# MaurizioFD/RecSys2019_DeepLearning_Evaluation

Hardware: NVIDIA B200
Metric: ItemKNN cosine top-K rows/sec (higher is better)
Workload: dtype i32 counts + f32

## Files before the change

### include/b200rec.h

```cpp
#ifndef B200REC_H_
#define B200REC_H_

#include <stdint.h>

#ifdef __cplusplus
extern "C" {
#endif

#define B200_OK 0
#define B200_E_INVALID (-1)
#define B200_E_CUDA (-2)
#define B200_E_NOMEM (-3)
#define B200_E_UNSUPPORTED (-4)

const char* b200_last_error(void);
int b200_version(void);
int64_t b200_launch_count(void);
int b200_device_info(char* name, int name_len, int* sm_count, int64_t* total_mem);

typedef struct b200_sim_s* b200_sim_t;

enum b200_sim_kind {
  B200_SIM_COSINE = 0,
  B200_SIM_ADJUSTED = 1,
  B200_SIM_ASYMMETRIC = 2,
  B200_SIM_PEARSON = 3,
  B200_SIM_JACCARD = 4,
  B200_SIM_DICE = 5,
  B200_SIM_TVERSKY = 6,
  B200_SIM_EUCLIDEAN = 7
};

int b200_sim_create(b200_sim_t* out, int64_t n_rows, int64_t n_cols, int64_t nnz, const int32_t* h_indptr,
                    const int32_t* h_indices, const float* h_data, int kind, int topK, float shrink,
                    int normalize, float asymmetric_alpha, float tversky_alpha, float tversky_beta,
                    const float* h_row_weights, void* stream);
int b200_sim_destroy(b200_sim_t h);

int b200_sim_create_scaled(b200_sim_t* out, int64_t n_rows, int64_t n_cols, int64_t nnz, const int32_t* h_indptr,
                           const int32_t* h_indices, const float* h_data, const float* h_A, const float* h_B,
                           int topK, void* stream);

enum b200_euclid_mode { B200_EUCLID_EXP = 0, B200_EUCLID_LIN = 1, B200_EUCLID_LOG = 2 };
int b200_sim_create_euclidean(b200_sim_t* out, int64_t n_rows, int64_t n_cols, int64_t nnz, const int32_t* h_indptr,
                              const int32_t* h_indices, const float* h_data, int topK, float shrink, int normalize,
                              int normalize_avg_row, int distance_mode, void* stream);

int b200_sim_info(b200_sim_t h, int* K, int* n_windows, int* window_cells, int* binary_path, int* signed_data);

int b200_sim_compute_device(b200_sim_t h, int start_col, int end_col, int32_t* d_idx, float* d_val,
                            int32_t* d_cnt, void* stream);
int b200_sim_compute(b200_sim_t h, int start_col, int end_col, int32_t* h_idx, float* h_val, int32_t* h_cnt);
int b200_sim_compute_peers_device(b200_sim_t h, int start_col, int end_col, int n_tables, void* const* d_tables,
                                  int64_t idx_offset, int64_t val_offset, int64_t cnt_offset, void* stream);
int b200_sim_compute_dense_device(b200_sim_t h, int start_col, int end_col, float* d_out, void* stream);

int b200_topk_table_to_csr_count(int n_cols, int K, const int32_t* d_cnt, int64_t* nnz_out, void* stream);
int b200_topk_table_to_csr_fill(int n_cols, int K, const int32_t* d_idx, const float* d_val,
                                const int32_t* d_cnt, int64_t nnz, int32_t* h_indptr, int32_t* h_indices,
                                float* h_data, void* stream);

int b200_sim_debug_set_cap(b200_sim_t h, int cap);

int b200_sim_debug_phase_cycles(b200_sim_t h, int enable, uint64_t* out8);

int b200_sim_debug_k1c(b200_sim_t h, int set_fail_every, int* enabled, int* ctas_per_sm, int* n_bitmap_cols, int* n_window_cols);

int b200_sim_last_kernel_ms(b200_sim_t h, float* ms);
int b200_sim_work(b200_sim_t h, int start_col, int end_col, int64_t* gathered_entries);
int b200_sim_col_work(b200_sim_t h, int64_t* out_n_cols);

typedef struct b200_mf_s* b200_mf_t;

enum b200_mf_algorithm { B200_MF_BPR = 0, B200_MF_FUNK_SVD = 1 };
enum b200_sgd_mode { B200_SGD = 0, B200_ADAGRAD = 1, B200_RMSPROP = 2, B200_ADAM = 3 };
enum b200_sampler { B200_SAMPLER_GLIBC = 0,
                    B200_SAMPLER_PHILOX = 1  };

int b200_mf_create(b200_mf_t* out, int64_t n_users, int64_t n_items, int64_t nnz, const int32_t* h_indptr,
                   const int32_t* h_indices, const float* h_data, int n_factors, int algorithm, int batch_size,
                   float negative_interactions_quota, float learning_rate, int use_bias, float user_reg,
                   float item_reg, float bias_reg, float positive_reg, float negative_reg, int sgd_mode,
                   float gamma, float beta_1, float beta_2, const double* h_user_factors,
                   const double* h_item_factors, int has_seed, uint32_t random_seed, int sampler, int hogwild);
int b200_mf_destroy(b200_mf_t h);
int b200_mf_epoch(b200_mf_t h, void* stream);
int b200_mf_set_user_shard(b200_mf_t h, int user_lo, int user_hi, int64_t samples_per_epoch, uint32_t stream_id);
int b200_mf_samples_last_epoch(b200_mf_t h, int64_t* n);
int b200_mf_get_samples(b200_mf_t h, int32_t* u, int32_t* i, int32_t* j, float* r);
int b200_mf_get_factors(b200_mf_t h, double* user_factors, double* item_factors, double* user_bias,
                        double* item_bias, double* global_bias);
int b200_mf_device_factors(b200_mf_t h, float** d_user_factors, float** d_item_factors);
int b200_mf_last_epoch_ms(b200_mf_t h, float* ms);
int b200_mf_delta_snapshot_device(const float* d_V, float* d_B, float* d_own, float* d_sum, int64_t n, void* stream);
int b200_mf_delta_apply_device(float* d_V, float* d_B, const float* d_sum, const float* d_own, int64_t n, void* stream);

typedef struct b200_asysvd_s* b200_asysvd_t;
int b200_asysvd_create(b200_asysvd_t* out, int64_t n_users, int64_t n_items, int64_t nnz, const int32_t* h_indptr,
                       const int32_t* h_indices, const float* h_data, int n_factors, double negative_interactions_quota,
                       float learning_rate, int use_bias, float user_reg, float item_reg, float bias_reg, int sgd_mode,
                       float gamma, float beta_1, float beta_2, const double* h_profile_factors,
                       const double* h_item_factors, int has_seed, uint32_t random_seed);
int b200_asysvd_destroy(b200_asysvd_t h);
int b200_asysvd_epoch(b200_asysvd_t h, void* stream);
int b200_asysvd_get_samples(b200_asysvd_t h, int32_t* u, int32_t* i, float* r);
int b200_asysvd_get_factors(b200_asysvd_t h, double* profile_factors, double* item_factors, double* user_bias,
                            double* item_bias, double* global_bias);
int b200_asysvd_last_epoch_ms(b200_asysvd_t h, float* ms);

typedef struct b200_slim_s* b200_slim_t;

int b200_slim_create(b200_slim_t* out, int64_t n_users, int64_t n_items, int64_t nnz, const int32_t* h_indptr,
                     const int32_t* h_indices, float learning_rate, float li_reg, float lj_reg, int symmetric,
                     int sgd_mode, float gamma, float beta_1, float beta_2, int has_seed, uint32_t random_seed,
                     int sampler, int hogwild);
int b200_slim_destroy(b200_slim_t h);
int b200_slim_epoch(b200_slim_t h, void* stream);
int b200_slim_get_samples(b200_slim_t h, int32_t* u, int32_t* i, int32_t* j);
int b200_slim_get_S_dense(b200_slim_t h, float* h_out, float* d_out);
int b200_slim_last_epoch_ms(b200_slim_t h, float* ms);
int b200_slim_enable_tree(b200_slim_t h, int topK);
int b200_slim_tree_prune(b200_slim_t h, int touch_diagonal, void* stream);
int b200_slim_create_sharded(b200_slim_t* out, int64_t n_users, int64_t n_items, int64_t nnz, const int32_t* h_indptr,
                             const int32_t* h_indices, float learning_rate, float li_reg, float lj_reg, int sgd_mode,
                             float gamma, float beta_1, float beta_2, uint32_t random_seed, int col_lo, int col_hi);
int b200_slim_shard_partial_device(b200_slim_t h, int64_t first, int n_batch, float* d_x, void* stream);
int b200_slim_shard_apply_device(b200_slim_t h, int64_t first, int n_batch, const float* d_x_sum, void* stream);
int b200_slim_shard_device(b200_slim_t h, float** d_S, int* col_lo, int* col_hi);

enum b200_topk_mode { B200_TOPK_NONZERO = 0, B200_TOPK_ZEROS_OUTRANK = 1,
                      B200_TOPK_NONZERO_DROP_LAST = 2 };
int b200_dense_topk_device(const float* d_matrix, int n, int K, int along_columns, int mode, int32_t* d_idx,
                           float* d_val, int32_t* d_cnt, void* stream);
int b200_dense_topk_rect_device(const float* d_matrix, int n_lines, int n_inner, int64_t stride_line, int64_t stride_inner,
                                int index_offset, int K, int mode, int32_t* d_idx, float* d_val, int32_t* d_cnt, void* stream);
int b200_sparse_topk_device(int n, const int32_t* d_ptr, const int32_t* d_line_idx, const float* d_vals, int K,
                            int mode, int32_t* d_idx, float* d_val, int32_t* d_cnt, void* stream);

int b200_score_spmm_device(const int32_t* d_users, int n_users_block, const int32_t* d_a_ptr, const int32_t* d_a_idx,
                           const float* d_a_val, const int32_t* d_b_ptr, const int32_t* d_b_idx, const float* d_b_val,
                           int n_out_cols, float* d_out, void* stream);
int b200_transpose_device(const float* d_in, int rows, int cols, float* d_out, void* stream);
int b200_score_mf_device(const int32_t* d_users, int n_users_block, const float* d_user_factors,
                         const float* d_item_factors_T, int n_factors, int n_items, const float* d_user_bias,
                         const float* d_item_bias, const float* d_global_bias, float* d_out, void* stream);
int b200_score_mask_device(const int32_t* d_users, int n_users_block, const int32_t* d_urm_ptr, const int32_t* d_urm_idx,
                           const unsigned char* d_items_keep, int n_items, float* d_scores, void* stream);
int b200_score_topn_device(const float* d_scores, int n_rows, int n_items, int cutoff, int32_t* d_items,
                           float* d_item_scores, void* stream);

int b200_slim_enet_device(const float* d_G, const float* d_diag, int n_items, int64_t n_users, double l1_ratio, double alpha,
                          int positive_only, int max_iter, float tol, float* d_coef_T, int32_t* d_n_iter, void* stream);

int b200_spd_inverse_device(float* d_A, int n_pad, float* d_work, void* stream);
int b200_debug_gemm_device(int version, int kind, int M, int N, int K, float alpha, const float* d_A, int lda,
                           const float* d_B, int ldb, float beta, float* d_C, int ldc, void* stream);
int b200_ease_from_gram_device(const float* d_G, int n_items, const int32_t* d_urm_indices, int64_t nnz, float l2_norm,
                               float* h_B, float* d_B, void* stream);

int b200_ials_half_epoch_device(const int32_t* d_rows, int n_solve, const int32_t* d_ptr, const int32_t* d_idx,
                                const float* d_conf, const double* d_Y, int n_other, int n_factors, double reg,
                                double* d_X, double* d_YtY_work, void* stream);

enum b200_weighting { B200_WEIGHT_BM25 = 0, B200_WEIGHT_TFIDF = 1 };
int b200_feature_weighting_device(int mode, int n_users, int n_items, int64_t nnz, const int32_t* d_indptr,
                                  const int32_t* d_indices, float* d_data, float K1, float B, void* stream);

enum b200_eval_slot {
  B200_EVAL_PRECISION = 0, B200_EVAL_PRECISION_RECALL_MIN_DEN = 1, B200_EVAL_RECALL = 2, B200_EVAL_MAP = 3,
  B200_EVAL_MAP_MIN_DEN = 4, B200_EVAL_MRR = 5, B200_EVAL_NDCG = 6, B200_EVAL_HIT_RATE = 7, B200_EVAL_ARHR = 8,
  B200_EVAL_NOVELTY = 9, B200_EVAL_AVERAGE_POPULARITY = 10, B200_EVAL_USERS_WITH_RECS = 11, B200_EVAL_N_USERS = 12,
  B200_EVAL_NACC = 16
};
int b200_eval_accumulate_device(const int32_t* d_users, int n_block, const int32_t* d_rec_items, const float* d_rec_scores,
                                int max_cutoff, const int32_t* d_test_ptr, const int32_t* d_test_idx,
                                const float* d_test_val, const int32_t* d_cutoffs, int n_cutoffs, const double* d_idcg,
                                const double* d_item_novelty, const double* d_item_pop_norm, int n_items, double* d_acc,
                                int32_t* d_rec_count, int32_t* d_hit_count, void* stream);

#ifdef __cplusplus
}
#endif
#endif
```

### recsys2019_deeplearning_evaluation_b200/csrc/sim_k1d.cuh

```cuda

constexpr int D_THREADS = 512;
constexpr int D_WARPS = D_THREADS / 32;
constexpr int D_ROWS = 4;
constexpr int D_TILE_LOG2 = 10;

struct K1DShared {
  int item, nbuf, cnt, adds, nibsum, tstop, chunk_end, chunk_cnt;
  int need, digit, bincnt, ncand, expect;
  u64 kor, kand;
  int hist[256];
};

__device__ __forceinline__ unsigned nib_ge3(unsigned w) { return (((w | (w >> 1)) >> 2) | (w & (w >> 1))) & 0x11111111u; }
__device__ __forceinline__ unsigned nib_eq2(unsigned w) { return (w >> 1) & ~w & ~(w >> 2) & ~(w >> 3) & 0x11111111u; }
__device__ __forceinline__ unsigned nib_eq1(unsigned w) { return w & ~(w >> 1) & ~(w >> 2) & ~(w >> 3) & 0x11111111u; }
__device__ __forceinline__ unsigned nib_level(unsigned w, int level) {
  return level >= 3 ? nib_ge3(w) : (level == 2 ? nib_eq2(w) : nib_eq1(w));
}
__device__ __forceinline__ int nib_sum(unsigned w) {
  const unsigned b = (w & 0x0F0F0F0Fu) + ((w >> 4) & 0x0F0F0F0Fu);
  return (int)__dp4a(b, 0x01010101u, 0u);
}

__device__ u64 d_select(u64* buf, int n, int K, K1DShared* ds, int* n_out) {
  const int tid = threadIdx.x;
  __syncthreads();
  if (n <= K) { *n_out = n; return 0ull; }
  {
    if (tid == 0) { ds->kor = 0ull; ds->kand = ~0ull; }
    __syncthreads();
    u64 o = 0ull, a = ~0ull;
    for (int q = tid; q < n; q += D_THREADS) { const u64 k = buf[q]; o |= k; a &= k; }
#pragma unroll
    for (int off = 16; off > 0; off >>= 1) { o |= __shfl_xor_sync(0xffffffffu, o, off); a &= __shfl_xor_sync(0xffffffffu, a, off); }
    if ((tid & 31) == 0) { atomicOr(&ds->kor, o); atomicAnd(&ds->kand, a); }
    __syncthreads();
  }
  const u64 diff = ds->kor ^ ds->kand;
  int pass = diff ? (63 - __clzll((long long)diff)) >> 3 : 0;
  u64 prefix = pass < 7 ? (ds->kor >> ((pass + 1) * 8)) << ((pass + 1) * 8) : 0ull;
  int need = K;
  const int one = n > 0 ? 1 : 0;
  for (; pass >= 0; --pass) {
    const int shift = pass * 8;
    if (tid < 256) ds->hist[tid] = 0;
    __syncthreads();
    for (int q = tid; q < n; q += D_THREADS) {
      const u64 k = buf[q];
      if (pass == 7 || (k >> (shift + 8)) == (prefix >> (shift + 8))) atomicAdd(&ds->hist[(int)((k >> shift) & 255ull)], one);
    }
    __syncthreads();
    if (tid < 32) {
      int c[8], local = 0;
#pragma unroll
      for (int b = 0; b < 8; ++b) { c[b] = ds->hist[255 - (tid * 8 + b)]; local += c[b]; }
      int incl = local;
#pragma unroll
      for (int off = 1; off < 32; off <<= 1) {
        const int t = __shfl_up_sync(0xffffffffu, incl, off);
        if (tid >= off) incl += t;
      }
      int cum = incl - local;
#pragma unroll
      for (int b = 0; b < 8; ++b) {
        if (cum < need && cum + c[b] >= need) { ds->digit = 255 - (tid * 8 + b); ds->need = need - cum; ds->bincnt = c[b]; }
        cum += c[b];
      }
    }
    __syncthreads();
    prefix |= ((u64)ds->digit) << shift;
    need = ds->need;
    const int bincnt = ds->bincnt;
    __syncthreads();
    if (bincnt == need) break;
  }
  const u64 thr = prefix;
  u64 keep[8];
#pragma unroll
  for (int q = 0; q < 8; ++q) {
    const int i = q * D_THREADS + tid;
    const u64 k = i < n ? buf[i] : 0ull;
    keep[q] = k >= thr ? k : 0ull;
  }
  if (tid == 0) ds->cnt = 0;
  __syncthreads();
#pragma unroll
  for (int q = 0; q < 8; ++q)
    if (keep[q]) buf[atomicAdd(&ds->cnt, 1)] = keep[q];
  __syncthreads();
  *n_out = ds->cnt;
  return thr;
}

template <int F>
__global__ void __launch_bounds__(D_THREADS, 2) sim_k1d_kernel(const KParams p) {
  extern __shared__ __align__(16) unsigned char smem_raw[];
  __shared__ K1DShared ds;
  const int tid = threadIdx.x, lane = tid & 31, warp = tid >> 5;
  const int W = p.bm_words;
  const int Wr = (p.n_cols + 7) >> 3;
  const int ntile = p.ntile;
  unsigned* acc = reinterpret_cast<unsigned*>(smem_raw);
  u64* buf = reinterpret_cast<u64*>(smem_raw + (size_t)W * 4);
  float* tbs = reinterpret_cast<float*>(buf + p.cap_d);
  int* tcnt = reinterpret_cast<int*>(tbs + ntile + 1);

  for (int i = tid; i < W; i += D_THREADS) acc[i] = 0u;
  for (int i = tid; i <= ntile; i += D_THREADS) tbs[i] = p.tbnd[i];
  for (int i = tid; i < ntile; i += D_THREADS) tcnt[i] = 0;
  long long prof_t = p.prof ? clock64() : 0;
  const int K = p.K;

  for (;;) {
    __syncthreads();
    if (tid == 0) { ds.item = atomicAdd(p.counter, 1); ds.nbuf = 0; ds.adds = 0; ds.nibsum = 0; ds.ncand = 0; }
    __syncthreads();
    const int item = ds.item;
    if (item >= p.n_range) break;
    const int4 wi = __ldg(p.worklist + item);
    const int col = wi.x, lc = wi.y, cs = wi.z, ce = wi.w;
    const size_t out_base = (size_t)lc * K;
    const float Ai = p.A[col];

    int expect = 0;
    for (int k0 = cs + warp * 32; k0 < ce; k0 += D_WARPS * 32) {
      const int nrows = min(32, ce - k0);
      int2 seg = make_int2(0, 0);
      if (lane < nrows) {
        seg = __ldg(p.csc_seg + k0 + lane);
        expect += 4 * (seg.y >> 2) - (seg.y & 3) - 1;
      }
      for (int r0 = 0; r0 < nrows; r0 += D_ROWS) {
        int4 v[D_ROWS];
        int rs[D_ROWS], rn[D_ROWS];
#pragma unroll
        for (int q = 0; q < D_ROWS; ++q) {
          const int r = r0 + q;
          rs[q] = __shfl_sync(0xffffffffu, seg.x, r & 31);
          rn[q] = r < nrows ? (__shfl_sync(0xffffffffu, seg.y, r & 31) >> 2) : 0;
          if (lane < rn[q]) v[q] = __ldg(reinterpret_cast<const int4*>(p.csr_idx1) + (size_t)rs[q] + lane);
        }
#pragma unroll
        for (int q = 0; q < D_ROWS; ++q) {
          int c0 = 0;
          for (;;) {
            if (c0 + lane < rn[q]) {
              const int jj[4] = {v[q].x, v[q].y, v[q].z, v[q].w};
#pragma unroll
              for (int c = 0; c < 4; ++c) {
                const int j = jj[c];
                if ((unsigned)j < (unsigned)p.n_cols && j != col) atomicAdd(&acc[j >> 3], 1u << ((j & 7) << 2));
              }
            }
            c0 += 32;
            if (c0 >= rn[q]) break;
            if (c0 + lane < rn[q]) v[q] = __ldg(reinterpret_cast<const int4*>(p.csr_idx1) + (size_t)rs[q] + c0 + lane);
          }
        }
      }
    }
    expect = __reduce_add_sync(0xffffffffu, expect);
    if (lane == 0 && expect) atomicAdd(&ds.adds, expect);
    __syncthreads();
    PROF_MARK(1);

    {
      int ns = 0;
      unsigned* cand = reinterpret_cast<unsigned*>(buf);
      const int cand_cap = p.cap_d;
      const uint4* acc4 = reinterpret_cast<const uint4*>(acc);
      for (int i4 = tid; i4 < ((Wr + 3) >> 2); i4 += D_THREADS) {
        const uint4 w4 = acc4[i4];
        if (!(w4.x | w4.y | w4.z | w4.w)) continue;
        const unsigned ww[4] = {w4.x, w4.y, w4.z, w4.w};
        unsigned bytes = 0u, any = 0u, m[4];
#pragma unroll
        for (int e = 0; e < 4; ++e) {
          bytes += (ww[e] & 0x0F0F0F0Fu) + ((ww[e] >> 4) & 0x0F0F0F0Fu);
          m[e] = nib_ge3(ww[e]);
          any |= m[e];
        }
        ns += (int)__dp4a(bytes, 0x01010101u, 0u);
        if (any) {
          const int c3 = __popc(m[0]) + __popc(m[1]) + __popc(m[2]) + __popc(m[3]);
          atomicAdd(&tcnt[(i4 * 4) >> (D_TILE_LOG2 - 3)], c3);
          int pos = atomicAdd(&ds.ncand, c3);
          if (pos + c3 <= cand_cap) {
#pragma unroll
            for (int e = 0; e < 4; ++e) {
              unsigned mm = m[e];
              while (mm) {
                const int q = (__ffs(mm) - 1) >> 2;
                mm &= mm - 1;
                cand[pos++] = ((unsigned)((i4 * 4 + e) * 8 + q) << 4) | ((ww[e] >> (q << 2)) & 15u);
              }
            }
          }
        }
      }
      ns = __reduce_add_sync(0xffffffffu, ns);
      if (lane == 0 && ns) atomicAdd(&ds.nibsum, ns);
    }
    __syncthreads();
    const bool forced = p.fail_every > 0 && (lc % p.fail_every) == 0;
    if (ds.nibsum != ds.adds || forced) {
      __syncthreads();
      if (tid == 0) p.redo[atomicAdd(p.fail, 1)] = lc;
      for (int i = tid; i < (W >> 2); i += D_THREADS) reinterpret_cast<int4*>(acc)[i] = make_int4(0, 0, 0, 0);
      for (int i = tid; i < ntile; i += D_THREADS) tcnt[i] = 0;
      continue;
    }
    PROF_MARK(2);

    u64 thr = 0ull;
    int n_have = 0;
    const int n3 = ds.ncand;
    const bool collected = n3 <= p.cap_d;
    if (collected) {
      const unsigned* cand = reinterpret_cast<const unsigned*>(buf);
      u64 keys[4];
#pragma unroll
      for (int q = 0; q < 4; ++q) {
        const int t = q * D_THREADS + tid;
        keys[q] = 0ull;
        if (t < n3) {
          const unsigned cd = cand[t];
          const int2 bn = __ldg(p.BN + (cd >> 4));
          const float sv = sim_value<F>(p, (float)(cd & 15u), Ai, __int_as_float(bn.x));
          if (sv > 0.f) keys[q] = (((u64)__float_as_uint(sv)) << 32) | (u64)(0xFFFFFFFFu - (unsigned)bn.y);
        }
      }
      __syncthreads();
#pragma unroll
      for (int q = 0; q < 4; ++q)
        if (keys[q]) buf[atomicAdd(&ds.nbuf, 1)] = keys[q];
      for (int i = tid; i < ntile; i += D_THREADS) tcnt[i] = 0;
      __syncthreads();
      n_have = ds.nbuf;
      if (n_have >= K) {
        const float fl = sim_value<F>(p, 3.f, Ai, tbs[ntile]) * (1.f - 1e-6f);
        if (fl > 0.f) thr = ((u64)__float_as_uint(fl)) << 32;
      }
      PROF_MARK(3);
    }
#pragma unroll 1
    for (int level = collected ? 2 : 3; level >= 1; --level) {
      int t_end = ntile;
      if (level < 3) {
        if (thr == 0ull) {
          t_end = ntile;
        } else {
          const float tsim = __uint_as_float((unsigned)(thr >> 32));
          if (tid == 0) ds.tstop = ntile;
          __syncthreads();
          for (int t = tid; t < ntile; t += D_THREADS)
            if (!(sim_value<F>(p, (float)level, Ai, tbs[t]) >= tsim)) atomicMin(&ds.tstop, t);
          __syncthreads();
          t_end = ds.tstop;
          __syncthreads();
        }
        if (t_end == 0) continue;
        const int w_end = min(Wr, t_end << (D_TILE_LOG2 - 3));
        for (int i = tid; i < w_end; i += D_THREADS) {
          const unsigned w = acc[i];
          if (!w) continue;
          const int c = __popc(nib_level(w, level));
          if (c) atomicAdd(&tcnt[i >> (D_TILE_LOG2 - 3)], c);
        }
        __syncthreads();
      }
      int t0 = 0;
      while (t0 < t_end) {
        if (tid == 0) {
          int t1 = t0, c = 0;
          while (t1 < t_end && n_have + c + tcnt[t1] <= p.cap_d) { c += tcnt[t1]; ++t1; }
          ds.chunk_end = t1;
          ds.chunk_cnt = c;
        }
        __syncthreads();
        const int t1 = ds.chunk_end;
        if (t1 == t0) {
          int kept;
          const u64 t2 = d_select(buf, n_have, K, &ds, &kept);
          thr = max(thr, t2);
          if (tid == 0) ds.nbuf = kept;
          n_have = kept;
          __syncthreads();
          continue;
        }
        if (ds.chunk_cnt > 0) {
          const int w_lo = t0 << (D_TILE_LOG2 - 3), w_hi = min(Wr, t1 << (D_TILE_LOG2 - 3));
          for (int i = w_lo + tid; i < w_hi; i += D_THREADS) {
            const unsigned w = acc[i];
            if (!w) continue;
            unsigned m = nib_level(w, level);
            while (m) {
              const int q = (__ffs(m) - 1) >> 2;
              m &= m - 1;
              const int j = i * 8 + q;
              const float d = (float)((w >> (q << 2)) & 15u);
              const int2 bn = __ldg(p.BN + j);
              const float sv = sim_value<F>(p, d, Ai, __int_as_float(bn.x));
              const u64 key = (((u64)__float_as_uint(sv)) << 32) | (u64)(0xFFFFFFFFu - (unsigned)bn.y);
              if (sv > 0.f && key >= thr) buf[atomicAdd(&ds.nbuf, 1)] = key;
            }
          }
        }
        __syncthreads();
        n_have = ds.nbuf;
        t0 = t1;
      }
      for (int i = tid; i < ntile; i += D_THREADS) tcnt[i] = 0;
      __syncthreads();
      if (n_have >= K) {
        if (level == 3 && thr == 0ull) {
          const float fl = sim_value<F>(p, 3.f, Ai, tbs[ntile]) * (1.f - 1e-6f);
          if (fl > 0.f) thr = ((u64)__float_as_uint(fl)) << 32;
        } else if (level == 2 && n_have > K) {
          int kept;
          const u64 t2 = d_select(buf, n_have, K, &ds, &kept);
          thr = max(thr, t2);
          if (tid == 0) ds.nbuf = kept;
          n_have = kept;
          __syncthreads();
        }
      }
      if (level == 3) PROF_MARK(3); else if (level == 2) PROF_MARK(4); else PROF_MARK(5);
    }

    {
      int kept;
      d_select(buf, n_have, K, &ds, &kept);
      n_have = kept;
    }
    for (int t = tid; t < n_have; t += D_THREADS) {
      const u64 k64 = buf[t];
      emit_entry(p, out_base + t, (int)(0xFFFFFFFFu - (unsigned)k64), __uint_as_float((unsigned)(k64 >> 32)));
    }
    for (int t = n_have + tid; t < K; t += D_THREADS) {
      emit_entry(p, out_base + t, -1, 0.f);
    }
    if (tid == 0) emit_count(p, lc, n_have);
    for (int i = tid; i < (W >> 2); i += D_THREADS) reinterpret_cast<int4*>(acc)[i] = make_int4(0, 0, 0, 0);
    PROF_MARK(6);
  }
}

__global__ void k1d_tile_bounds_kernel(const int2* __restrict__ BN, int n_cols, int ntile, float* tb) {
  const int t = blockIdx.x * blockDim.x + threadIdx.x;
  if (t > ntile) return;
  tb[t] = __int_as_float(BN[min(t << D_TILE_LOG2, n_cols - 1)].x);
}

__global__ void k1d_csc_seg_kernel(const int* __restrict__ csc_idx, const int* __restrict__ split1, const int* __restrict__ csr_ptr,
                                   long long nnz, int2* seg) {
  for (long long q = blockIdx.x * (long long)blockDim.x + threadIdx.x; q < nnz; q += (long long)gridDim.x * blockDim.x) {
    const int u = csc_idx[q];
    const int s = split1[2 * (size_t)u], e = split1[2 * (size_t)u + 1];
    const int len = csr_ptr[u + 1] - csr_ptr[u];
    seg[q] = make_int2(s >> 2, (((e - s) >> 2) << 2) | ((e - s) - len));
  }
}
```

### recsys2019_deeplearning_evaluation_b200/csrc/sim_topk.cu

```cuda
#include <cub/device/device_radix_sort.cuh>
#include <cub/device/device_scan.cuh>
#include <cub/device/device_segmented_sort.cuh>

#include <stdlib.h>

#include <algorithm>
#include <cmath>
#include <vector>

#include "common.cuh"

namespace b200 {
namespace sim {

typedef unsigned long long u64;

constexpr int THREADS = 1024;
constexpr int NWARPS = THREADS / 32;
constexpr int STAGE_INTS = 3072;
constexpr int SPMAX = 5;
constexpr int HBINS = 4096;
constexpr int SBINS = 2048;
#ifndef B200_SELT
#define B200_SELT 256
#endif
constexpr int SELT = B200_SELT;
#ifndef B200_UB
#define B200_UB 2
#endif
constexpr int UB = B200_UB;
#ifndef B200_PREFETCH
#define B200_PREFETCH 0
#endif
#ifndef B200_GUESS
#define B200_GUESS 0
#endif
constexpr int MAXTILES = 16;
#define B200_MAX_PEERS 8

enum Formula { F_PROD = 0, F_NONORM = 1, F_JACCARD = 2, F_DICE = 3, F_TVERSKY = 4, F_SCALE = 5, F_EUCLID = 6 };

struct KParams {
  int n_cols, K, n_win, win, cap, cap_alloc;
  int acc_cells;
  int lpu_log2;
  float se;
  float shrink_div;
  float ta, tb;
  const int* __restrict__ csr_ptr;
  const int2* __restrict__ csr_ent;
  const int* __restrict__ csr_idx;
  const int* __restrict__ split;
  const int* __restrict__ csc_ptr;
  const int2* __restrict__ csc_ent;
  const int* __restrict__ csc_idx;
  const float* __restrict__ A;
  const int2* __restrict__ BN;
  const float* __restrict__ tileB;
  const int* __restrict__ old2new;
  int col_begin, n_range;
  const int* __restrict__ order;
  int* counter;
  int n_out;
  int* o_idx[B200_MAX_PEERS];
  float* o_val[B200_MAX_PEERS];
  int* o_cnt[B200_MAX_PEERS];
  int signed_data;
  int eu_mode, eu_norm, eu_signed;
  float eu_div, eu_shrink;
  float* dense_out;
  int bm_words, cap_d, fail_every, ntile;
  const float* __restrict__ tbnd;
  const int* __restrict__ csr_idx1;
  const int2* __restrict__ csc_seg;
  const int4* __restrict__ worklist;
  int* redo;
  int* fail;
  const int* n_range_dev;
  unsigned long long* prof;
};

__device__ __forceinline__ void emit_entry(const KParams& p, size_t pos, int idx, float val) {
#pragma unroll 1
  for (int r = 0; r < p.n_out; ++r) { p.o_idx[r][pos] = idx; p.o_val[r][pos] = val; }
}
__device__ __forceinline__ void emit_count(const KParams& p, int row, int n) {
#pragma unroll 1
  for (int r = 0; r < p.n_out; ++r) p.o_cnt[r][row] = n;
}

template <int F>
__device__ __forceinline__ float sim_value(const KParams& p, float d, float a, float b) {
  if (F == F_PROD) return d / (a * b + p.se);
  if (F == F_NONORM) return d / p.shrink_div;
  if (F == F_JACCARD) return d / (a + b - d + p.se);
  if (F == F_DICE) return d / (a + b + p.se);
  if (F == F_SCALE) return d * a * b;
  return d / (d + (a - d) * p.ta + (b - d) * p.tb + p.se);
}

__device__ __forceinline__ float euclid_sim(const KParams& p, float d2, float sq_i, float sq_j) {
  float d = d2;
  if (p.eu_norm) {
    const float den = sqrtf(sq_i) * sqrtf(sq_j);
    if (den != 0.f) d = d / den;
  }
  d = d / p.eu_div;
  if (d > 0.f) d = sqrtf(d);
  const float g = p.eu_mode == 0 ? expf(d) : (p.eu_mode == 1 ? d : logf(d + 1.f));
  return 1.f / ((g + p.eu_shrink) + 1e-9f);
}

template <int F>
__device__ __forceinline__ float dot_threshold(const KParams& p, float t, float a, float b_lo, float b_hi) {
  float r = 3.4e38f;
#pragma unroll
  for (int e = 0; e < 2; ++e) {
    const float b = e ? b_hi : b_lo;
    float v;
    if (F == F_PROD) v = t * (a * b + p.se);
    else if (F == F_NONORM) v = t * p.shrink_div;
    else if (F == F_JACCARD) v = t * (a + b + p.se) / (1.f + t);
    else if (F == F_DICE) v = t * (a + b + p.se);
    else if (F == F_SCALE) v = (a * b > 0.f) ? t / (a * b) : 3.4e38f;
    else {
      const float den = 1.f - t * (1.f - p.ta - p.tb);
      v = den > 1e-6f ? t * (a * p.ta + b * p.tb + p.se) / den : 0.f;
    }
    r = fminf(r, v);
  }
  return r > 0.f ? r * (1.f - 1e-5f) : 0.f;
}

template <int F>
__device__ __forceinline__ float dot_threshold_sure(const KParams& p, float t, float a, float b_lo, float b_hi) {
  float r = 0.f;
#pragma unroll
  for (int e = 0; e < 2; ++e) {
    const float b = e ? b_hi : b_lo;
    float v;
    if (F == F_PROD) v = t * (a * b + p.se);
    else if (F == F_NONORM) v = t * p.shrink_div;
    else if (F == F_JACCARD) v = t * (a + b + p.se) / (1.f + t);
    else if (F == F_DICE) v = t * (a + b + p.se);
    else if (F == F_SCALE) v = (a * b > 0.f) ? t / (a * b) : 3.4e38f;
    else {
      const float den = 1.f - t * (1.f - p.ta - p.tb);
      v = (den > 1e-6f && p.ta >= 0.f && p.tb >= 0.f) ? t * (a * p.ta + b * p.tb + p.se) / den : 3.4e38f;
    }
    r = fmaxf(r, v);
  }
  return r < 1e37f ? r * (1.f + 1e-4f) + 1e-30f : 3.4e38f;
}

template <int F>
__device__ __forceinline__ float lower_bound_scale(const KParams& p, float a, float b_lo, float b_hi) {
  const float b = fmaxf(b_lo, b_hi);
  float den;
  if (F == F_SCALE) return a * fminf(b_lo, b_hi) * (1.f - 1e-5f);
  if (F == F_PROD) den = a * b + p.se;
  else if (F == F_NONORM) den = p.shrink_div;
  else if (F == F_JACCARD || F == F_DICE) den = a + b + p.se;
  else {
    if (p.ta < 0.f || p.tb < 0.f) return 0.f;
    den = a * fmaxf(0.f, 1.f - p.ta - p.tb) + a * p.ta + b * p.tb + p.se;
  }
  return den > 0.f ? (1.f - 1e-5f) / den : 0.f;
}

#define PROF_MARK(ph)                                                        \
  do {                                                                      \
    if (p.prof && threadIdx.x == 0) {                                       \
      const long long _t = clock64();                                       \
      atomicAdd(p.prof + (ph), (unsigned long long)(_t - prof_t));          \
      prof_t = _t;                                                          \
    }                                                                       \
  } while (0)

template <bool NEG>
__device__ __forceinline__ unsigned key32_of(float v) {
  return NEG ? ~__float_as_uint(v) : __float_as_uint(v);
}

struct Shared {
  int col;
  float guess;
  int next;
  int nbuf;
  int overflow;
  int npos, nneg;
  int digit, need, bincnt;
  int b0;
  int cnt;
  unsigned kmin, kmax;
  u64 sel_thr;
  int warp_tot[NWARPS];
  float dthr[MAXTILES];
  float lbs[MAXTILES];
  unsigned k2[MAXTILES];
};

constexpr int LB_BASE = (127 - 40) << 6;
__device__ __forceinline__ int lb_bin(const float lb) {
  return min(max((int)(__float_as_uint(lb) >> 17) - LB_BASE, 0), HBINS - 1);
}
__device__ __forceinline__ unsigned lb_bin_floor_bits(const int b) { return ((unsigned)(b + LB_BASE)) << 17; }

__device__ __forceinline__ unsigned half_ge_mask(const uint4 v, const unsigned k2) {
  const unsigned M = 0x80008000u;
  return (((v.x + k2) & M) >> 15) | (((v.y + k2) & M) >> 14) | (((v.z + k2) & M) >> 13) | (((v.w + k2) & M) >> 12);
}
__device__ __forceinline__ unsigned half_k2(const float dthr) {
  const unsigned t = dthr <= 1.f ? 1u : (dthr >= 32768.f ? 0x8000u : (unsigned)ceilf(dthr));
  return (0x8000u - t) * 0x10001u;
}

__device__ __forceinline__ void bar_sel() { asm volatile("bar.sync 1, %0;" ::"n"(SELT) : "memory"); }

__device__ __forceinline__ int block_suffix_excl(int v, int* warp_tot) {
  const int lane = threadIdx.x & 31, warp = threadIdx.x >> 5;
  int incl = v;
#pragma unroll
  for (int off = 1; off < 32; off <<= 1) {
    int t = __shfl_down_sync(0xffffffffu, incl, off);
    if (lane + off < 32) incl += t;
  }
  if (lane == 0) warp_tot[warp] = incl;
  __syncthreads();
  int above = 0;
  for (int w = warp + 1; w < NWARPS; ++w) above += warp_tot[w];
  __syncthreads();
  return above + incl - v;
}

__device__ void select_group(u64* buf, int n, int K, Shared* sh, int* hist) {
  const int tid = threadIdx.x, lane = tid & 31, warp = tid >> 5;
  constexpr int SW = SELT / 32;
  for (int i = tid; i < SBINS; i += SELT) hist[i] = 0;
  if (tid == 0) { sh->kmin = 0xFFFFFFFFu; sh->kmax = 0u; sh->cnt = 0; }
  bar_sel();
  {
    unsigned mn = 0xFFFFFFFFu, mx = 0u;
    int valid = 0;
    for (int q = tid; q < n; q += SELT) {
      const u64 k = buf[q];
      if (k) {
        const unsigned h = (unsigned)(k >> 32);
        mn = min(mn, h);
        mx = max(mx, h);
        ++valid;
      }
    }
    mn = __reduce_min_sync(0xffffffffu, mn);
    mx = __reduce_max_sync(0xffffffffu, mx);
    valid = __reduce_add_sync(0xffffffffu, valid);
    if (lane == 0) { atomicMin(&sh->kmin, mn); atomicMax(&sh->kmax, mx); atomicAdd(&sh->cnt, valid); }
  }
  bar_sel();
  const int valid = sh->cnt;
  u64 thr = 0;
  if (valid > K) {
    u64 base = ((u64)sh->kmin) << 32;
    const u64 top = (((u64)sh->kmax) << 32) | 0xFFFFFFFFull;
    int width = 64 - __clzll((long long)(top - base));
    int need = K;
    while (true) {
      const int shift = max(0, width - 11);
      for (int q = tid; q < n; q += SELT) {
        const u64 k = buf[q];
        const u64 off = k - base;
        if (k >= base && k != 0ull && (width >= 64 || (off >> width) == 0ull)) atomicAdd(&hist[(int)(off >> shift)], 1);
      }
      bar_sel();
      int c[SBINS / SELT], local = 0;
#pragma unroll
      for (int b = 0; b < SBINS / SELT; ++b) {
        c[b] = hist[tid * (SBINS / SELT) + b];
        hist[tid * (SBINS / SELT) + b] = 0;
        local += c[b];
      }
      int incl = local;
#pragma unroll
      for (int off = 1; off < 32; off <<= 1) {
        const int t = __shfl_down_sync(0xffffffffu, incl, off);
        if (lane + off < 32) incl += t;
      }
      if (lane == 0) sh->warp_tot[warp] = incl;
      bar_sel();
      int cum = incl - local;
      for (int w = warp + 1; w < SW; ++w) cum += sh->warp_tot[w];
#pragma unroll
      for (int b = SBINS / SELT - 1; b >= 0; --b) {
        if (cum < need && cum + c[b] >= need) { sh->digit = tid * (SBINS / SELT) + b; sh->need = need - cum; sh->bincnt = c[b]; }
        cum += c[b];
      }
      bar_sel();
      base += ((u64)sh->digit) << shift;
      need = sh->need;
      const int bincnt = sh->bincnt;
      width = shift;
      bar_sel();
      if (bincnt == need || shift == 0) break;
    }
    thr = base;
  }
  if (tid == 0) sh->cnt = 0;
  u64 keep[16];
  const int rounds = (n + SELT - 1) / SELT;
  for (int r0 = 0; r0 < rounds; r0 += 16) {
#pragma unroll
    for (int q = 0; q < 16; ++q) {
      const int i = (r0 + q) * SELT + tid;
      const u64 k = (r0 + q < rounds && i < n) ? buf[i] : 0ull;
      keep[q] = (k != 0ull && k >= thr) ? k : 0ull;
    }
    bar_sel();
#pragma unroll
    for (int q = 0; q < 16; ++q)
      if (keep[q]) buf[atomicAdd(&sh->cnt, 1)] = keep[q];
    bar_sel();
  }
  if (tid == 0) sh->sel_thr = thr;
}

__device__ __forceinline__ u64 block_select(u64* buf, int n, int K, Shared* sh, int* hist, int* n_out) {
  __syncthreads();
  if (threadIdx.x < SELT) select_group(buf, n, K, sh, hist);
  __syncthreads();
  *n_out = sh->cnt;
  return sh->sel_thr;
}

template <bool BINARY, bool PACK>
__device__ __forceinline__ bool load_cells(const void* acc, int iv, float* d) {
  if (PACK) {
    const int4 v = reinterpret_cast<const int4*>(acc)[iv];
    if ((v.x | v.y | v.z | v.w) == 0) return false;
    d[0] = (float)(v.x & 0xFFFF); d[1] = (float)((unsigned)v.x >> 16); d[2] = (float)(v.y & 0xFFFF); d[3] = (float)((unsigned)v.y >> 16);
    d[4] = (float)(v.z & 0xFFFF); d[5] = (float)((unsigned)v.z >> 16); d[6] = (float)(v.w & 0xFFFF); d[7] = (float)((unsigned)v.w >> 16);
    return true;
  } else if (BINARY) {
    const int4 v = reinterpret_cast<const int4*>(acc)[iv];
    if ((v.x | v.y | v.z | v.w) == 0) return false;
    d[0] = (float)v.x; d[1] = (float)v.y; d[2] = (float)v.z; d[3] = (float)v.w;
    return true;
  } else {
    const float4 v = reinterpret_cast<const float4*>(acc)[iv];
    if (v.x == 0.f && v.y == 0.f && v.z == 0.f && v.w == 0.f) return false;
    d[0] = v.x; d[1] = v.y; d[2] = v.z; d[3] = v.w;
    return true;
  }
}

template <bool BINARY, bool PACK>
__device__ __forceinline__ void store_cells(void* acc, int iv, const float* k) {
  if (PACK) {
    reinterpret_cast<int4*>(acc)[iv] = make_int4((int)k[0] | ((int)k[1] << 16), (int)k[2] | ((int)k[3] << 16),
                                                 (int)k[4] | ((int)k[5] << 16), (int)k[6] | ((int)k[7] << 16));
  } else if (BINARY) {
    reinterpret_cast<int4*>(acc)[iv] = make_int4((int)k[0], (int)k[1], (int)k[2], (int)k[3]);
  } else {
    reinterpret_cast<float4*>(acc)[iv] = make_float4(k[0], k[1], k[2], k[3]);
  }
}

__device__ __forceinline__ void prefetch_l2_range(const void* base, long long byte_lo, long long byte_hi) {
  const char* b = reinterpret_cast<const char*>(base);
  for (long long o = byte_lo & ~127ll; o < byte_hi; o += 128)
    asm volatile("prefetch.global.L2 [%0];" ::"l"(b + o));
}

template <bool BINARY>
__device__ __forceinline__ void prefetch_column(const KParams& p, int c_next, int q, int nthr) {
  if (c_next >= p.n_range) return;
  const int lc = p.order ? p.order[c_next] : c_next;
  const int col = p.old2new[p.col_begin + lc];
  const int cs = p.csc_ptr[col], ce = p.csc_ptr[col + 1];
  for (int t = cs + q; t < ce; t += nthr) {
    const int u = BINARY ? p.csc_idx[t] : p.csc_ent[t].x;
    if (p.n_win == 1 && !BINARY) {
      const int s0 = p.csr_ptr[u], e0 = p.csr_ptr[u + 1];
      prefetch_l2_range(p.csr_ent, 8ll * s0, 8ll * e0);
    } else {
      const int* sp = p.split + (size_t)u * (p.n_win + 1);
      const int s0 = sp[0], e0 = sp[p.n_win];
      if (BINARY) prefetch_l2_range(p.csr_idx, 4ll * s0, 4ll * e0);
      else prefetch_l2_range(p.csr_ent, 8ll * s0, 8ll * e0);
    }
  }
}

template <int F, bool BINARY, bool PACK, bool NEG>
__device__ void process_column(const KParams& p, int col, int target, int out_base, unsigned char* smem_raw,
                               Shared* sh, const float* s_tileB, int* n_emitted) {
  const int tid = threadIdx.x, lane = tid & 31, warp = tid >> 5;
  float* accf = reinterpret_cast<float*>(smem_raw);
  int* acci = reinterpret_cast<int*>(smem_raw);
  u64* buf = reinterpret_cast<u64*>(smem_raw + (size_t)p.acc_cells * 4);
  int* hist = reinterpret_cast<int*>(buf);
  int* stage = reinterpret_cast<int*>(buf + p.cap_alloc);
  int* shist_stage = stage;
  bool staged_valid = false;

  const int cs = p.csc_ptr[col], ce = p.csc_ptr[col + 1];
  const float Ai = p.A[col];
  long long prof_t = p.prof ? clock64() : 0;
  u64 thr = 0;
  int nbuf = 0;
  if (tid == 0) { sh->nbuf = 0; if (!NEG) { sh->npos = 0; sh->nneg = 0; } }

  const bool all_splits = (p.n_win + 1 <= SPMAX) && (ce - cs <= STAGE_INTS / (p.n_win + 2));
  const int sp_stride = all_splits ? (p.n_win + 1) : 2;
  const int colchunk = STAGE_INTS / (1 + sp_stride);
  float* sm_x = reinterpret_cast<float*>(stage);
  int* sm_sp = stage + colchunk;
  const int lpu = 1 << p.lpu_log2, upw = 32 >> p.lpu_log2;
  const int sub = lane & (lpu - 1), uslot = lane >> p.lpu_log2;
  __syncthreads();

  if (F == F_EUCLID) {
    const int lo = p.eu_norm ? max(0, col - target) : 0;
    const int hi = p.eu_norm ? min(p.n_cols, col + target + 1) : min(p.n_cols, target + 1);
    for (int t = lo + tid; t < hi; t += THREADS) {
      u64 key = 0ull;
      if (t != col) {
        const int2 bn = __ldg(p.BN + t);
        const float b = __int_as_float(bn.x);
        const float dmax2 = p.eu_signed ? (Ai + b) + 2.f * sqrtf(Ai) * sqrtf(b) : (Ai + b);
        const float sv = euclid_sim(p, dmax2, Ai, b);
        if (sv > 0.f) key = (((u64)__float_as_uint(sv)) << 32) | (u64)(0xFFFFFFFFu - (unsigned)bn.y);
      }
      buf[t - lo] = key;
    }
    int kept;
    const u64 t0 = block_select(buf, hi - lo, target, sh, acci, &kept);
    if (t0) thr = ((u64)__float_as_uint(__uint_as_float((unsigned)(t0 >> 32)) * (1.f - 1e-5f))) << 32;
    if (tid == 0) sh->nbuf = 0;
    __syncthreads();
  }

  for (int w = 0; w < p.n_win; ++w) {
    const int win_lo = w * p.win;
    const int win_n = min(p.win, p.n_cols - win_lo);
    constexpr int CPV = PACK ? 8 : 4;
    const int winv = (win_n + CPV - 1) / CPV;
    const int ntiles = (winv + THREADS - 1) / THREADS;
    const float* tB = s_tileB + w * (MAXTILES + 1);
    int* accw_i = acci - win_lo;
    float* accw_f = accf - win_lo;
    unsigned* accw_u = reinterpret_cast<unsigned*>(acci) - (win_lo >> 1);

    for (int k0 = cs; k0 < ce; k0 += colchunk) {
      const int n = min(colchunk, ce - k0);
      if (!all_splits || !staged_valid) {
        staged_valid = true;
        __syncthreads();
        for (int t = tid; t < n; t += THREADS) {
          int u;
          if (BINARY) {
            u = p.csc_idx[k0 + t];
          } else {
            const int2 e = p.csc_ent[k0 + t];
            u = e.x;
            sm_x[t] = __int_as_float(e.y);
          }
          if (p.n_win == 1 && !BINARY) {
            sm_sp[t * 2] = p.csr_ptr[u];
            sm_sp[t * 2 + 1] = p.csr_ptr[u + 1];
          } else if (all_splits) {
            const int* sp = p.split + (size_t)u * (p.n_win + 1);
            for (int q = 0; q <= p.n_win; ++q) sm_sp[t * sp_stride + q] = sp[q];
          } else {
            const int* sp = p.split + (size_t)u * (p.n_win + 1) + w;
            sm_sp[t * 2] = sp[0];
            sm_sp[t * 2 + 1] = sp[1];
          }
        }
        __syncthreads();
      }
      PROF_MARK(0);
      const int spo = all_splits ? w : 0;
      for (int t0 = warp * upw; t0 < n; t0 += NWARPS * upw * UB) {
        int s[UB], e[UB], a0[UB];
        float x[UB];
        int mych = 0;
#pragma unroll
        for (int k = 0; k < UB; ++k) {
          const int t = t0 + k * NWARPS * upw + uslot;
          if (t < n) {
            s[k] = sm_sp[t * sp_stride + spo];
            e[k] = sm_sp[t * sp_stride + spo + 1];
            x[k] = BINARY ? 1.f : sm_x[t];
          } else {
            s[k] = 0; e[k] = 0; x[k] = 0.f;
          }
          a0[k] = BINARY ? s[k] : (s[k] & ~1);
          mych = max(mych, BINARY ? ((e[k] - a0[k]) >> 2) : ((e[k] - a0[k] + 1) >> 1));
        }
        const int maxch = __reduce_max_sync(0xffffffffu, mych);
        for (int c0 = 0; c0 < maxch; c0 += lpu) {
          const int ch = c0 + sub;
          int4 v[UB];
#pragma unroll
          for (int k = 0; k < UB; ++k) {
            const int g = a0[k] + ch * (BINARY ? 4 : 2);
            v[k] = make_int4(-1, -1, -1, -1);
            if (g < e[k]) v[k] = BINARY ? __ldg(reinterpret_cast<const int4*>(p.csr_idx + g))
                                        : __ldg(reinterpret_cast<const int4*>(p.csr_ent + g));
          }
#pragma unroll
          for (int k = 0; k < UB; ++k) {
            const int g = a0[k] + ch * (BINARY ? 4 : 2);
            if (BINARY) {
              if (g < e[k]) {
                const int jj[4] = {v[k].x, v[k].y, v[k].z, v[k].w};
#pragma unroll
                for (int c = 0; c < 4; ++c) {
                  if (PACK) atomicAdd(&accw_u[jj[c] >> 1], (jj[c] & 1) ? 65536u : 1u);
                  else atomicAdd(&accw_i[jj[c]], 1);
                }
              }
            } else {
              if (g >= s[k] && g < e[k]) atomicAdd(&accw_f[v[k].x], x[k] * __int_as_float(v[k].y));
              if (g + 1 >= s[k] && g + 1 < e[k]) atomicAdd(&accw_f[v[k].z], x[k] * __int_as_float(v[k].w));
            }
          }
        }
      }
    }
    __syncthreads();
    if (tid == 0 && col >= win_lo && col < win_lo + win_n) {
      const int c = col - win_lo;
      if (PACK) acci[c >> 1] &= (c & 1) ? 0x0000FFFF : (int)0xFFFF0000; else acci[c] = 0;
    }
    __syncthreads();
    PROF_MARK(1);
    if (p.dense_out) {
      float* orow = p.dense_out + (size_t)out_base * p.n_cols;
      for (int c = tid; c < win_n; c += THREADS) {
        const float d = PACK ? (float)(((unsigned)acci[c >> 1] >> ((c & 1) * 16)) & 0xFFFFu) : (BINARY ? (float)acci[c] : accf[c]);
        if (d != 0.f) {
          const int2 bn = __ldg(p.BN + win_lo + c);
          orow[bn.y] = sim_value<F>(p, d, Ai, __int_as_float(bn.x));
        }
      }
      __syncthreads();
      for (int iv = tid; iv < winv; iv += THREADS) reinterpret_cast<int4*>(acci)[iv] = make_int4(0, 0, 0, 0);
      __syncthreads();
      continue;
    }

    if (F == F_EUCLID) {
      int ub = sh->nbuf;
      __syncthreads();
      for (int c0 = 0; c0 < win_n; c0 += THREADS) {
        if (ub + THREADS > p.cap) {
          ub = sh->nbuf;
          __syncthreads();
          if (ub + THREADS > p.cap) {
            int kept;
            staged_valid = false;
            thr = max(thr, block_select(buf, ub, target, sh, shist_stage, &kept));
            if (tid == 0) sh->nbuf = kept;
            ub = kept;
            __syncthreads();
          }
        }
        ub += THREADS;
        const int c = c0 + tid;
        if (c < win_n && win_lo + c != col) {
          const float d = PACK ? (float)(((unsigned)acci[c >> 1] >> ((c & 1) * 16)) & 0xFFFFu) : (BINARY ? (float)acci[c] : accf[c]);
          const int2 bn = __ldg(p.BN + win_lo + c);
          const float b = __int_as_float(bn.x);
          const float sv = euclid_sim(p, (b + Ai) - 2.f * d, Ai, b);
          const u64 key = (((u64)__float_as_uint(sv)) << 32) | (u64)(0xFFFFFFFFu - (unsigned)bn.y);
          if (sv > 0.f && key >= thr) buf[atomicAdd(&sh->nbuf, 1)] = key;
        }
        __syncthreads();
      }
      for (int iv = tid; iv < winv; iv += THREADS) reinterpret_cast<int4*>(acci)[iv] = make_int4(0, 0, 0, 0);
      __syncthreads();
      nbuf = sh->nbuf;
      if (w == p.n_win - 1) {
        int kept;
        thr = max(thr, block_select(buf, nbuf, target, sh, acci, &kept));
        if (tid == 0) sh->nbuf = kept;
        nbuf = kept;
        __syncthreads();
      }
      PROF_MARK(3);
      continue;
    }

    nbuf = sh->nbuf;
#if B200_GUESS
    if (F != F_EUCLID && !NEG && thr == 0 && nbuf == 0 && win_n > 2 * target && sh->guess > 0.f) {
      const float g = sh->guess;
      if (tid == 0) sh->cnt = 0;
      if (tid < ntiles) {
        const float dt = dot_threshold_sure<F>(p, g, Ai, tB[tid], tB[tid + 1]);
        sh->dthr[tid] = dt;
        if (PACK) sh->k2[tid] = half_k2(dt);
      }
      __syncthreads();
      int sure = 0;
      for (int iv = tid; iv < winv; iv += THREADS) {
        if (PACK) {
          sure += __popc(half_ge_mask(reinterpret_cast<const uint4*>(acci)[iv], sh->k2[iv / THREADS]));
        } else {
          float d[CPV];
          if (!load_cells<BINARY, PACK>(acci, iv, d)) continue;
          const float dthr = sh->dthr[iv / THREADS];
#pragma unroll
          for (int c = 0; c < CPV; ++c) sure += (d[c] > 0.f && d[c] >= dthr) ? 1 : 0;
        }
      }
      sure = __reduce_add_sync(0xffffffffu, sure);
      if (lane == 0 && sure) atomicAdd(&sh->cnt, sure);
      __syncthreads();
      if (sh->cnt >= target) thr = ((u64)__float_as_uint(g)) << 32;
      __syncthreads();
    }
#endif
    if (!NEG && thr == 0 && nbuf == 0 && win_n > 2 * target) {
      for (int i = tid; i < HBINS; i += THREADS) hist[i] = 0;
      if (tid == 0) sh->b0 = -1;
      if (tid < ntiles) sh->lbs[tid] = lower_bound_scale<F>(p, Ai, tB[tid], tB[tid + 1]);
      __syncthreads();
      if (PACK) {
        for (int iv0 = warp * 32; iv0 < winv; iv0 += THREADS) {
          const int iv = iv0 + lane;
          const float sc = sh->lbs[iv0 / THREADS];
          uint4 v = make_uint4(0u, 0u, 0u, 0u);
          if (iv < winv) v = reinterpret_cast<const uint4*>(acci)[iv];
          const int n1 = __popc(half_ge_mask(v, 0x7FFF7FFFu)), n2 = __popc(half_ge_mask(v, 0x7FFE7FFEu));
          unsigned m3 = half_ge_mask(v, 0x7FFD7FFDu);
          const int n3 = __popc(m3);
          while (m3) {
            const int b = __ffs(m3) - 1;
            m3 &= m3 - 1;
            const int q = b & 3;
            const unsigned wq = q == 0 ? v.x : (q == 1 ? v.y : (q == 2 ? v.z : v.w));
            const float lb = (float)((b >> 4) ? (wq >> 16) : (wq & 0xFFFFu)) * sc;
            if (lb > 0.f) atomicAdd(&hist[lb_bin(lb)], 1);
          }
          const int c1 = __reduce_add_sync(0xffffffffu, n1 - n2), c2 = __reduce_add_sync(0xffffffffu, n2 - n3);
          if (lane == 0 && sc > 0.f) {
            if (c1) atomicAdd(&hist[lb_bin(sc)], c1);
            if (c2) atomicAdd(&hist[lb_bin(2.f * sc)], c2);
          }
        }
      } else {
        for (int iv = tid; iv < winv; iv += THREADS) {
          const float sc = sh->lbs[iv / THREADS];
          float d[CPV];
          if (!load_cells<BINARY, PACK>(acci, iv, d)) continue;
#pragma unroll
          for (int c = 0; c < CPV; ++c) {
            const float lb = d[c] * sc;
            if (lb > 0.f) atomicAdd(&hist[lb_bin(lb)], 1);
          }
        }
      }
      __syncthreads();
      int hh[HBINS / THREADS], local = 0;
#pragma unroll
      for (int b = 0; b < HBINS / THREADS; ++b) { hh[b] = hist[tid * (HBINS / THREADS) + b]; local += hh[b]; }
      int cum = block_suffix_excl(local, sh->warp_tot);
#pragma unroll
      for (int b = HBINS / THREADS - 1; b >= 0; --b) {
        if (cum < target && cum + hh[b] >= target) sh->b0 = tid * (HBINS / THREADS) + b;
        cum += hh[b];
      }
      __syncthreads();
      const int b0 = sh->b0;
      if (b0 > 0) thr = ((u64)lb_bin_floor_bits(b0)) << 32;
      __syncthreads();
    }
    PROF_MARK(2);

    bool first = true;
    while (true) {
      const int nbuf_old = sh->nbuf;
      __syncthreads();
      if (tid == 0) sh->overflow = 0;
      if (tid < ntiles) {
        const float dt = (!NEG && thr) ? dot_threshold<F>(p, __uint_as_float((unsigned)(thr >> 32)), Ai, tB[tid], tB[tid + 1]) : 0.f;
        sh->dthr[tid] = dt;
        if (PACK) sh->k2[tid] = half_k2(dt);
      }
      int cpos = 0, cneg = 0;
      const bool count_signs = !NEG && first && p.signed_data;
      __syncthreads();
      for (int iv = tid; iv < winv; iv += THREADS) {
        const float dthr = sh->dthr[iv / THREADS];
        if (PACK && !NEG) {
          const uint4 v = reinterpret_cast<const uint4*>(acci)[iv];
          unsigned m = half_ge_mask(v, sh->k2[iv / THREADS]);
          reinterpret_cast<int4*>(acci)[iv] = make_int4(0, 0, 0, 0);
          while (m) {
            const int b = __ffs(m) - 1;
            m &= m - 1;
            const int q = b & 3, hf = b >> 4;
            const unsigned wq = q == 0 ? v.x : (q == 1 ? v.y : (q == 2 ? v.z : v.w));
            const unsigned cntv = hf ? (wq >> 16) : (wq & 0xFFFFu);
            const int pos = atomicAdd(&sh->nbuf, 1);
            if (pos < p.cap)
              buf[pos] = (((u64)__float_as_uint((float)cntv)) << 32) | (u64)(unsigned)(win_lo + iv * CPV + 2 * q + hf);
            else {
              sh->overflow = 1;
              reinterpret_cast<unsigned short*>(acci)[iv * CPV + 2 * q + hf] = (unsigned short)cntv;
            }
          }
          continue;
        }
        float d[CPV];
        if (!load_cells<BINARY, PACK>(acci, iv, d)) continue;
        if (count_signs) {
#pragma unroll
          for (int c = 0; c < CPV; ++c) { cpos += d[c] > 0.f; cneg += d[c] < 0.f; }
        }
        float keepv[CPV];
        float dmax = NEG ? -d[0] : d[0];
#pragma unroll
        for (int c = 0; c < CPV; ++c) { keepv[c] = 0.f; dmax = fmaxf(dmax, NEG ? -d[c] : d[c]); }
        if (dmax > 0.f && dmax >= dthr) {
#pragma unroll
          for (int c = 0; c < CPV; ++c) {
            const float dd = d[c];
            if (NEG ? (dd < 0.f) : (dd > 0.f && dd >= dthr)) {
              const int pos = atomicAdd(&sh->nbuf, 1);
              if (pos < p.cap)
                buf[pos] = (((u64)__float_as_uint(dd)) << 32) | (u64)(unsigned)(win_lo + iv * CPV + c);
              else { sh->overflow = 1; keepv[c] = dd; }
            }
          }
        }
        store_cells<BINARY, PACK>(acci, iv, keepv);
      }
      if (count_signs) {
#pragma unroll
        for (int off = 16; off > 0; off >>= 1) {
          cpos += __shfl_xor_sync(0xffffffffu, cpos, off);
          cneg += __shfl_xor_sync(0xffffffffu, cneg, off);
        }
        if (lane == 0) { if (cpos) atomicAdd(&sh->npos, cpos); if (cneg) atomicAdd(&sh->nneg, cneg); }
      }
      first = false;
      __syncthreads();
      PROF_MARK(3);
      const int n_end = min(sh->nbuf, p.cap);
      const bool overflow = sh->overflow != 0;
      for (int e = nbuf_old + tid; e < n_end; e += THREADS) {
        const u64 rec = buf[e];
        const int j = (int)(unsigned)rec;
        const float dd = __uint_as_float((unsigned)(rec >> 32));
        const int2 bn = __ldg(p.BN + j);
        const float sv = sim_value<F>(p, dd, Ai, __int_as_float(bn.x));
        const u64 key = (((u64)key32_of<NEG>(sv)) << 32) | (u64)(0xFFFFFFFFu - (unsigned)bn.y);
        buf[e] = (key >= thr && (NEG ? (sv < 0.f) : (sv > 0.f))) ? key : 0ull;
      }
      nbuf = n_end;
      __syncthreads();
      if (tid == 0) sh->nbuf = nbuf;
      PROF_MARK(4);
      if (!overflow) break;
      int kept;
      staged_valid = false;
      thr = max(thr, block_select(buf, nbuf, target, sh, shist_stage, &kept));
      if (tid == 0) sh->nbuf = kept;
      __syncthreads();
    }
    __syncthreads();
    nbuf = sh->nbuf;
    if (nbuf > p.cap / 2 || w == p.n_win - 1) {
      int kept;
#if B200_PREFETCH
      if (w == p.n_win - 1) {
        __syncthreads();
        if (tid < SELT) select_group(buf, nbuf, target, sh, acci);
        else prefetch_column<BINARY>(p, sh->next, tid - SELT, THREADS - SELT);
        __syncthreads();
        kept = sh->cnt;
        thr = max(thr, sh->sel_thr);
      } else
#endif
      thr = max(thr, block_select(buf, nbuf, target, sh, acci, &kept));
      if (tid == 0) sh->nbuf = kept;
      nbuf = kept;
      __syncthreads();
    }
    PROF_MARK(5);
  }

#if B200_GUESS
  if (!NEG && tid == 0) sh->kmin = 0xFFFFFFFFu;
  __syncthreads();
#endif
  for (int t = tid; t < nbuf; t += THREADS) {
    const u64 k = buf[t];
    const unsigned hi = (unsigned)(k >> 32);
#if B200_GUESS
    if (!NEG) atomicMin(&sh->kmin, hi);
#endif
    emit_entry(p, (size_t)out_base + t, (int)(0xFFFFFFFFu - (unsigned)k), __uint_as_float(NEG ? ~hi : hi));
  }
  *n_emitted = nbuf;
  __syncthreads();
#if B200_GUESS
  if (!NEG && tid == 0) sh->guess = (F != F_EUCLID && nbuf >= target) ? 0.9f * __uint_as_float(sh->kmin) : 0.f;
#endif
  PROF_MARK(6);
}

template <int F, bool BINARY, bool PACK>
__global__ void __launch_bounds__(THREADS, 1) sim_topk_kernel(const KParams p) {
  extern __shared__ __align__(16) unsigned char smem_raw[];
  __shared__ Shared sh;
  const int tid = threadIdx.x;
  float* s_tileB = reinterpret_cast<float*>(smem_raw + (size_t)p.acc_cells * 4 + (size_t)p.cap_alloc * 8 +
                                            (size_t)STAGE_INTS * 4);
  {
    const int4 z = make_int4(0, 0, 0, 0);
    for (int i4 = tid; i4 < (p.acc_cells >> 2); i4 += THREADS) reinterpret_cast<int4*>(smem_raw)[i4] = z;
    for (int i = tid; i < p.n_win * (MAXTILES + 1); i += THREADS) s_tileB[i] = p.tileB[i];
    if (tid == 0) sh.guess = 0.f;
  }
  __syncthreads();
  const int n_range = p.n_range_dev ? *p.n_range_dev : p.n_range;
#if B200_PREFETCH
  if (tid == 0) sh.next = atomicAdd(p.counter, 1);
#endif
  while (true) {
#if B200_PREFETCH
    __syncthreads();
    const int c = sh.next;
    __syncthreads();
    if (c >= n_range) break;
    if (tid == 0) sh.next = atomicAdd(p.counter, 1);
#else
    if (tid == 0) sh.col = atomicAdd(p.counter, 1);
    __syncthreads();
    const int c = sh.col;
    if (c >= n_range) break;
#endif
    const int lc = p.order ? p.order[c] : c;
    const int col = p.old2new[p.col_begin + lc];
    const int out_base_row = lc;
    int n_out = 0;
    if (p.dense_out) {
      process_column<F, BINARY, PACK, false>(p, col, p.K, out_base_row, smem_raw, &sh, s_tileB, &n_out);
      __syncthreads();
      continue;
    }
    process_column<F, BINARY, PACK, false>(p, col, p.K, out_base_row * p.K, smem_raw, &sh, s_tileB, &n_out);
    if (p.signed_data && n_out < p.K) {
      const int npos = sh.npos, nneg = sh.nneg;
      const int nzero = p.n_cols - npos - nneg;
      const int m = p.K - n_out - nzero;
      __syncthreads();
      if (m > 0 && nneg > 0) {
        int n_neg_out = 0;
        process_column<F, BINARY, PACK, true>(p, col, m, out_base_row * p.K + n_out, smem_raw, &sh, s_tileB, &n_neg_out);
        n_out += n_neg_out;
      }
    }
    for (int t = n_out + tid; t < p.K; t += THREADS) {
      emit_entry(p, (size_t)out_base_row * p.K + t, -1, 0.f);
    }
    if (tid == 0) emit_count(p, out_base_row, n_out);
    __syncthreads();
  }
}

__global__ void tile_bounds_kernel(const int2* __restrict__ BN, int n_cols, int n_win, int win, int tile, float* tileB) {
  const int g = blockIdx.x * blockDim.x + threadIdx.x;
  if (g >= n_win * (MAXTILES + 1)) return;
  const int w = g / (MAXTILES + 1), t = g % (MAXTILES + 1);
  const int win_lo = w * win, win_n = min(win, n_cols - win_lo);
  const int j = min(win_lo + t * tile, win_lo + win_n - 1);
  tileB[g] = __int_as_float(BN[j].x);
}

#include "sim_k1d.cuh"

__global__ void flags_kernel(const float* __restrict__ data, long long nnz, int* flags) {
  int f = 0;
  for (long long i = blockIdx.x * (long long)blockDim.x + threadIdx.x; i < nnz; i += (long long)gridDim.x * blockDim.x) {
    float v = data[i];
    if (v != 1.0f) f |= 1;
    if (v < 0.f) f |= 2;
  }
  f = __reduce_or_sync(0xffffffffu, f);
  if ((threadIdx.x & 31) == 0 && f) atomicOr(flags, f);
}

__global__ void fill_ones_kernel(float* data, long long nnz) {
  for (long long i = blockIdx.x * (long long)blockDim.x + threadIdx.x; i < nnz; i += (long long)gridDim.x * blockDim.x)
    data[i] = 1.0f;
}

__global__ void row_center_kernel(const int* __restrict__ ptr, float* data, int n_rows) {
  const int warp = (blockIdx.x * blockDim.x + threadIdx.x) >> 5, lane = threadIdx.x & 31;
  if (warp >= n_rows) return;
  const int s = ptr[warp], e = ptr[warp + 1];
  if (e <= s) return;
  double sum = 0.0;
  for (int q = s + lane; q < e; q += 32) sum += (double)data[q];
#pragma unroll
  for (int off = 16; off > 0; off >>= 1) sum += __shfl_xor_sync(0xffffffffu, sum, off);
  const double mean = sum / (double)(e - s);
  for (int q = s + lane; q < e; q += 32) data[q] = (float)((double)data[q] - mean);
}

__global__ void col_accum_kernel(const int* __restrict__ idx, const float* __restrict__ data, long long nnz,
                                 double* colsum, double* colsq, int* colcnt) {
  for (long long i = blockIdx.x * (long long)blockDim.x + threadIdx.x; i < nnz; i += (long long)gridDim.x * blockDim.x) {
    const int j = idx[i];
    const double v = (double)data[i];
    if (colsum) atomicAdd(colsum + j, v);
    if (colsq) atomicAdd(colsq + j, v * v);
    if (colcnt) atomicAdd(colcnt + j, 1);
  }
}

__global__ void col_center_kernel(const int* __restrict__ idx, float* data, long long nnz,
                                  const double* __restrict__ colsum, const int* __restrict__ colcnt) {
  for (long long i = blockIdx.x * (long long)blockDim.x + threadIdx.x; i < nnz; i += (long long)gridDim.x * blockDim.x) {
    const int j = idx[i];
    const int c = colcnt[j];
    if (c > 0) data[i] = (float)((double)data[i] - colsum[j] / (double)c);
  }
}

__global__ void norms_kernel(const double* __restrict__ colsq, int n_cols, int mode, float alpha, float* A, float* B,
                             unsigned* Bkey, int* iota) {
  const int j = blockIdx.x * blockDim.x + threadIdx.x;
  if (j >= n_cols) return;
  const double sq = colsq[j];
  float a, b;
  if (mode == 0) {
    a = b = (float)sq;
  } else if (mode == 1) {
    a = b = (float)sqrt(sq);
  } else {
    const double n = sqrt(sq) + 1e-6;
    a = (float)pow(n, 2.0 * (double)alpha);
    b = (float)pow(n, 2.0 * (1.0 - (double)alpha));
  }
  A[j] = a;
  B[j] = b;
  Bkey[j] = __float_as_uint(b);
  iota[j] = j;
}

__global__ void scaled_keys_kernel(const float* __restrict__ B, int n_cols, unsigned* Bkey, int* iota) {
  const int j = blockIdx.x * blockDim.x + threadIdx.x;
  if (j >= n_cols) return;
  Bkey[j] = __float_as_uint(fmaxf(B[j], 0.f));
  iota[j] = j;
}

__global__ void renumber_kernel(const int* __restrict__ new2old, const float* __restrict__ A_old,
                                const float* __restrict__ B_old, const int* __restrict__ cnt_old, int n_cols,
                                int* old2new, float* A_new, int2* BN, int* cnt_new) {
  const int jn = blockIdx.x * blockDim.x + threadIdx.x;
  if (jn >= n_cols) return;
  const int jo = new2old[jn];
  old2new[jo] = jn;
  A_new[jn] = A_old[jo];
  BN[jn] = make_int2(__float_as_int(B_old[jo]), jo);
  cnt_new[jn] = cnt_old[jo];
}

__global__ void relabel_kernel(const int* __restrict__ idx_old, const int* __restrict__ old2new, long long nnz, int* idx_new) {
  for (long long i = blockIdx.x * (long long)blockDim.x + threadIdx.x; i < nnz; i += (long long)gridDim.x * blockDim.x)
    idx_new[i] = old2new[idx_old[i]];
}

__global__ void rowid_iota_kernel(const int* __restrict__ ptr, int n_rows, int* rowid, int* iota) {
  const int warp = (blockIdx.x * blockDim.x + threadIdx.x) >> 5, lane = threadIdx.x & 31;
  if (warp >= n_rows) return;
  const int s = ptr[warp], e = ptr[warp + 1];
  for (int q = s + lane; q < e; q += 32) { rowid[q] = warp; iota[q] = q; }
}

__global__ void build_csr_ent_kernel(const int* __restrict__ idx, const float* __restrict__ data, long long nnz, int2* ent) {
  for (long long i = blockIdx.x * (long long)blockDim.x + threadIdx.x; i < nnz; i += (long long)gridDim.x * blockDim.x)
    ent[i] = make_int2(idx[i], __float_as_int(data[i]));
}

__global__ void build_csc_kernel(const int* __restrict__ perm, const int* __restrict__ rowid,
                                 const float* __restrict__ data, const float* __restrict__ row_w, long long nnz,
                                 int2* ent, int* idx_only) {
  for (long long q = blockIdx.x * (long long)blockDim.x + threadIdx.x; q < nnz; q += (long long)gridDim.x * blockDim.x) {
    const int pp = perm[q];
    const int u = rowid[pp];
    if (idx_only) {
      idx_only[q] = u;
    } else {
      float x = data ? data[pp] : 1.0f;
      if (row_w) x *= row_w[u];
      ent[q] = make_int2(u, __float_as_int(x));
    }
  }
}

__global__ void split_kernel(const int* __restrict__ ptr, const int* __restrict__ idx, int n_rows, int n_win,
                             int win, int* split) {
  const long long g = blockIdx.x * (long long)blockDim.x + threadIdx.x;
  const long long total = (long long)n_rows * (n_win + 1);
  if (g >= total) return;
  const int u = (int)(g / (n_win + 1)), w = (int)(g % (n_win + 1));
  int lo = ptr[u], hi = ptr[u + 1];
  if (w == 0) { split[g] = lo; return; }
  if (w == n_win) { split[g] = hi; return; }
  const int bound = w * win;
  while (lo < hi) {
    const int mid = (lo + hi) >> 1;
    if (idx[mid] < bound) lo = mid + 1; else hi = mid;
  }
  split[g] = lo;
}

__global__ void seg_len_kernel(const int* __restrict__ split, long long n_seg, int n_win, int* len4) {
  const long long g = blockIdx.x * (long long)blockDim.x + threadIdx.x;
  if (g >= n_seg) return;
  const long long u = g / n_win;
  const int w = (int)(g % n_win);
  const int* sp = split + u * (n_win + 1) + w;
  len4[g] = (sp[1] - sp[0] + 3) & ~3;
}

__global__ void seg_pad_kernel(const int* __restrict__ split, const int* __restrict__ idx, const int* __restrict__ poff,
                               long long n_seg, int n_win, int win, int total, int* idx_pad, int* split_pad) {
  const long long g = (blockIdx.x * (long long)blockDim.x + threadIdx.x) >> 3;
  const int l = threadIdx.x & 7;
  if (g >= n_seg) return;
  const long long u = g / n_win;
  const int w = (int)(g % n_win);
  const int* sp = split + u * (n_win + 1) + w;
  const int s = sp[0], n = sp[1] - sp[0], n4 = (n + 3) & ~3, o = poff[g];
  for (int t = l; t < n4; t += 8) idx_pad[o + t] = t < n ? idx[s + t] : (w + 1) * win;
  if (l == 0) {
    split_pad[u * (n_win + 1) + w] = o;
    if (w == n_win - 1) split_pad[u * (n_win + 1) + n_win] = o + n4;
  }
}

__global__ void col_work_kernel(const int* __restrict__ csc_ptr, const int* __restrict__ csc_idx,
                                const int2* __restrict__ csc_ent, const int* __restrict__ csr_ptr, int n_cols,
                                unsigned long long* work) {
  const int warp = (blockIdx.x * blockDim.x + threadIdx.x) >> 5, lane = threadIdx.x & 31;
  if (warp >= n_cols) return;
  unsigned long long s = 0;
  for (int q = csc_ptr[warp] + lane; q < csc_ptr[warp + 1]; q += 32) {
    const int u = csc_idx ? csc_idx[q] : csc_ent[q].x;
    s += (unsigned long long)(csr_ptr[u + 1] - csr_ptr[u]);
  }
#pragma unroll
  for (int off = 16; off > 0; off >>= 1) s += __shfl_xor_sync(0xffffffffu, s, off);
  if (lane == 0) work[warp] = s;
}

}
}

using namespace b200;
using namespace b200::sim;

struct b200_sim_s {
  int n_rows = 0, n_cols = 0;
  long long nnz = 0;
  int kind = 0, K = 0, normalize = 0;
  float shrink = 0.f, asym_alpha = 0.5f, ta = 1.f, tb = 1.f;
  int formula = F_PROD;
  bool binary = false, signed_data = false;
  bool pack = false;
  bool allow_pack = true;
  int acc_words = 0;
  int eu_mode = 1, eu_norm = 0, eu_avg = 0;
  bool scaled = false;
  const float* h_A = nullptr;
  const float* h_B = nullptr;
  int n_win = 1, win = 0, cap = 2048, cap_alloc = 2048;
  size_t smem_bytes = 0;
  int n_sm = 0;
  DevBuf<int> csr_ptr, csr_idx, csc_ptr, csc_idx, split, old2new;
  DevBuf<int2> csr_ent, csc_ent, BN;
  DevBuf<float> A, tileB;
  int lpu_log2 = 3;
  bool want_k1c = true, k1c = false;
  DevBuf<int> csr_idx1, fail;
  DevBuf<int2> csc_seg;
  DevBuf<float> tbnd;
  DevBuf<int4> worklist;
  int bm_words = 0, cap_d = 0, fail_every = 0, ctas_per_sm = 0, ntile = 0;
  size_t smem1_bytes = 0;
  double k1c_lambda = 0.75;
  int k1c_min_cols = 32768;
  std::vector<int> h_old2new, h_csc_ptr;
  int n_sparse_last = 0, n_dense_last = 0;
  std::vector<unsigned long long> h_work;
  DevBuf<int> counter, order;
  std::vector<int> h_order;
  int order_lo = -1, order_hi = -1;
  DevBuf<unsigned long long> prof;
  bool prof_on = false;
  cudaEvent_t ev0 = nullptr, ev1 = nullptr;
  bool timed = false;
};

namespace {

constexpr int GRID1D = 148 * 8;

typedef void (*sim_kernel_t)(const KParams);
template <int F>
sim_kernel_t kernel_of(bool binary, bool pack) {
  if (binary && pack) return sim_topk_kernel<F, true, true>;
  if (binary) return sim_topk_kernel<F, true, false>;
  return sim_topk_kernel<F, false, false>;
}
sim_kernel_t kernel_for(int formula, bool binary, bool pack) {
  switch (formula) {
    case F_PROD: return kernel_of<F_PROD>(binary, pack);
    case F_NONORM: return kernel_of<F_NONORM>(binary, pack);
    case F_JACCARD: return kernel_of<F_JACCARD>(binary, pack);
    case F_DICE: return kernel_of<F_DICE>(binary, pack);
    case F_SCALE: return sim_topk_kernel<F_SCALE, false, false>;
    case F_EUCLID: return kernel_of<F_EUCLID>(binary, pack);
    default: return kernel_of<F_TVERSKY>(binary, pack);
  }
}

sim_kernel_t k1d_kernel_for(int formula) {
  switch (formula) {
    case F_PROD: return sim_k1d_kernel<F_PROD>;
    case F_NONORM: return sim_k1d_kernel<F_NONORM>;
    case F_JACCARD: return sim_k1d_kernel<F_JACCARD>;
    case F_DICE: return sim_k1d_kernel<F_DICE>;
    default: return sim_k1d_kernel<F_TVERSKY>;
  }
}

int bits_for(long long n) {
  int b = 1;
  while ((1ll << b) < n) ++b;
  return b;
}

void build(b200_sim_s* h, const int32_t* h_indptr, const int32_t* h_indices, const float* h_data,
           const float* h_row_weights, cudaStream_t st) {
  const int n_rows = h->n_rows, n_cols = h->n_cols;
  const long long nnz = h->nnz;
  const size_t nnz1 = (size_t)std::max<long long>(nnz, 1);
  h->n_sm = sm_count();
  B200_CUDA(cudaEventCreate(&h->ev0));
  B200_CUDA(cudaEventCreate(&h->ev1));

  h->csr_ptr.alloc((size_t)n_rows + 1);
  DevBuf<int> idx_old(nnz1);
  DevBuf<float> data(nnz1);
  B200_CUDA(cudaMemcpyAsync(h->csr_ptr.get(), h_indptr, sizeof(int) * ((size_t)n_rows + 1), cudaMemcpyHostToDevice, st));
  if (nnz) {
    B200_CUDA(cudaMemcpyAsync(idx_old.get(), h_indices, sizeof(int) * (size_t)nnz, cudaMemcpyHostToDevice, st));
    B200_CUDA(cudaMemcpyAsync(data.get(), h_data, sizeof(float) * (size_t)nnz, cudaMemcpyHostToDevice, st));
  }
  DevBuf<float> row_w;
  if (h_row_weights) {
    row_w.alloc((size_t)n_rows);
    B200_CUDA(cudaMemcpyAsync(row_w.get(), h_row_weights, sizeof(float) * (size_t)n_rows, cudaMemcpyHostToDevice, st));
  }

  const bool set_kind = !h->scaled && (h->kind == B200_SIM_JACCARD || h->kind == B200_SIM_DICE || h->kind == B200_SIM_TVERSKY);
  DevBuf<double> colsum((size_t)n_cols), colsq((size_t)n_cols);
  DevBuf<int> colcnt((size_t)n_cols);
  B200_CUDA(cudaMemsetAsync(colsum.get(), 0, sizeof(double) * (size_t)n_cols, st));
  B200_CUDA(cudaMemsetAsync(colsq.get(), 0, sizeof(double) * (size_t)n_cols, st));
  B200_CUDA(cudaMemsetAsync(colcnt.get(), 0, sizeof(int) * (size_t)n_cols, st));
  if (nnz && !h->scaled) {
    if (set_kind) {
      fill_ones_kernel<<<GRID1D, 256, 0, st>>>(data.get(), nnz); count_launch();
    } else if (h->kind == B200_SIM_ADJUSTED) {
      row_center_kernel<<<div_up((long long)n_rows * 32, 256), 256, 0, st>>>(h->csr_ptr.get(), data.get(), n_rows); count_launch();
    } else if (h->kind == B200_SIM_PEARSON) {
      col_accum_kernel<<<GRID1D, 256, 0, st>>>(idx_old.get(), data.get(), nnz, colsum.get(), nullptr, colcnt.get()); count_launch();
      col_center_kernel<<<GRID1D, 256, 0, st>>>(idx_old.get(), data.get(), nnz, colsum.get(), colcnt.get()); count_launch();
      B200_CUDA(cudaMemsetAsync(colcnt.get(), 0, sizeof(int) * (size_t)n_cols, st));
    }
  }
  DevBuf<int> flags(1);
  B200_CUDA(cudaMemsetAsync(flags.get(), 0, sizeof(int), st));
  if (nnz) { flags_kernel<<<GRID1D, 256, 0, st>>>(data.get(), nnz, flags.get()); count_launch(); }
  int hflags = 0;
  B200_CUDA(cudaMemcpyAsync(&hflags, flags.get(), sizeof(int), cudaMemcpyDeviceToHost, st));
  if (nnz) { col_accum_kernel<<<GRID1D, 256, 0, st>>>(idx_old.get(), data.get(), nnz, nullptr, colsq.get(), colcnt.get()); count_launch(); }
  DevBuf<float> A_old((size_t)n_cols), B_old((size_t)n_cols);
  DevBuf<unsigned> Bkey((size_t)n_cols), Bkey_sorted((size_t)n_cols);
  DevBuf<int> col_iota((size_t)n_cols), new2old((size_t)n_cols), cnt_new((size_t)n_cols);
  if (h->scaled) {
    B200_CUDA(cudaMemcpyAsync(A_old.get(), h->h_A, sizeof(float) * (size_t)n_cols, cudaMemcpyHostToDevice, st));
    B200_CUDA(cudaMemcpyAsync(B_old.get(), h->h_B, sizeof(float) * (size_t)n_cols, cudaMemcpyHostToDevice, st));
    scaled_keys_kernel<<<div_up(n_cols, 256), 256, 0, st>>>(B_old.get(), n_cols, Bkey.get(), col_iota.get());
  } else {
    const int norm_mode = (set_kind || h->kind == B200_SIM_EUCLIDEAN) ? 0 : (h->kind == B200_SIM_ASYMMETRIC ? 2 : 1);
    norms_kernel<<<div_up(n_cols, 256), 256, 0, st>>>(colsq.get(), n_cols, norm_mode, h->asym_alpha, A_old.get(), B_old.get(),
                                                      Bkey.get(), col_iota.get());
  }
  count_launch();

  {
    size_t tb = 0;
    B200_CUDA(cub::DeviceRadixSort::SortPairs(nullptr, tb, Bkey.get(), Bkey_sorted.get(), col_iota.get(), new2old.get(), n_cols, 0, 32, st));
    DevBuf<unsigned char> tmp(tb + 16);
    B200_CUDA(cub::DeviceRadixSort::SortPairs(tmp.get(), tb, Bkey.get(), Bkey_sorted.get(), col_iota.get(), new2old.get(), n_cols, 0, 32, st));
    count_launch(4);
    B200_CUDA(cudaStreamSynchronize(st));
  }
  h->old2new.alloc((size_t)n_cols);
  h->A.alloc((size_t)n_cols);
  h->BN.alloc((size_t)n_cols);
  renumber_kernel<<<div_up(n_cols, 256), 256, 0, st>>>(new2old.get(), A_old.get(), B_old.get(), colcnt.get(), n_cols,
                                                       h->old2new.get(), h->A.get(), h->BN.get(), cnt_new.get());
  count_launch();
  B200_CUDA(cudaStreamSynchronize(st));
  h->signed_data = (hflags & 2) != 0;
  h->binary = ((hflags & 1) == 0) && !h_row_weights && !h->scaled;

  h->csr_idx.alloc(nnz1 + 8);
  DevBuf<float> data_sorted(nnz1);
  if (nnz) {
    DevBuf<int> idx_new(nnz1);
    relabel_kernel<<<GRID1D, 256, 0, st>>>(idx_old.get(), h->old2new.get(), nnz, idx_new.get()); count_launch();
    size_t tb = 0;
    B200_CUDA(cub::DeviceSegmentedSort::SortPairs(nullptr, tb, idx_new.get(), h->csr_idx.get(), data.get(), data_sorted.get(),
                                                  (long long)nnz, (long long)n_rows, h->csr_ptr.get(), h->csr_ptr.get() + 1, st));
    DevBuf<unsigned char> tmp(tb + 16);
    B200_CUDA(cub::DeviceSegmentedSort::SortPairs(tmp.get(), tb, idx_new.get(), h->csr_idx.get(), data.get(), data_sorted.get(),
                                                  (long long)nnz, (long long)n_rows, h->csr_ptr.get(), h->csr_ptr.get() + 1, st));
    count_launch(3);
    B200_CUDA(cudaStreamSynchronize(st));
  }
  idx_old.release();
  data.release();

  h->csc_ptr.alloc((size_t)n_cols + 1);
  B200_CUDA(cudaMemsetAsync(h->csc_ptr.get(), 0, sizeof(int) * ((size_t)n_cols + 1), st));
  {
    size_t tb = 0;
    B200_CUDA(cub::DeviceScan::InclusiveSum(nullptr, tb, cnt_new.get(), h->csc_ptr.get() + 1, n_cols, st));
    DevBuf<unsigned char> tmp(tb + 16);
    B200_CUDA(cub::DeviceScan::InclusiveSum(tmp.get(), tb, cnt_new.get(), h->csc_ptr.get() + 1, n_cols, st));
    count_launch(2);
    B200_CUDA(cudaStreamSynchronize(st));
  }
  if (nnz) {
    DevBuf<int> rowid(nnz1), iota(nnz1), keys_out(nnz1), perm(nnz1);
    rowid_iota_kernel<<<div_up((long long)n_rows * 32, 256), 256, 0, st>>>(h->csr_ptr.get(), n_rows, rowid.get(), iota.get()); count_launch();
    size_t tb = 0;
    const int end_bit = bits_for(n_cols);
    B200_CUDA(cub::DeviceRadixSort::SortPairs(nullptr, tb, h->csr_idx.get(), keys_out.get(), iota.get(), perm.get(), (int)nnz, 0, end_bit, st));
    DevBuf<unsigned char> tmp(tb + 16);
    B200_CUDA(cub::DeviceRadixSort::SortPairs(tmp.get(), tb, h->csr_idx.get(), keys_out.get(), iota.get(), perm.get(), (int)nnz, 0, end_bit, st));
    count_launch(4);
    if (h->binary) {
      h->csc_idx.alloc((size_t)nnz);
      build_csc_kernel<<<GRID1D, 256, 0, st>>>(perm.get(), rowid.get(), data_sorted.get(), nullptr, nnz, nullptr, h->csc_idx.get());
    } else {
      h->csc_ent.alloc((size_t)nnz);
      h->csr_ent.alloc((size_t)nnz + 8);
      build_csc_kernel<<<GRID1D, 256, 0, st>>>(perm.get(), rowid.get(), h->scaled ? nullptr : data_sorted.get(), row_w.get(), nnz, h->csc_ent.get(), nullptr);
      build_csr_ent_kernel<<<GRID1D, 256, 0, st>>>(h->csr_idx.get(), data_sorted.get(), nnz, h->csr_ent.get()); count_launch();
    }
    count_launch();
    B200_CUDA(cudaStreamSynchronize(st));
  }

  if (h->scaled) {
    h->formula = F_SCALE;
  } else if (set_kind) {
    h->formula = h->kind == B200_SIM_JACCARD ? F_JACCARD : (h->kind == B200_SIM_DICE ? F_DICE : F_TVERSKY);
  } else if (h->kind == B200_SIM_EUCLIDEAN) {
    h->formula = F_EUCLID;
  } else {
    h->formula = h->normalize ? F_PROD : F_NONORM;
  }

  int dev = 0, max_smem = 0;
  B200_CUDA(cudaGetDevice(&dev));
  B200_CUDA(cudaDeviceGetAttribute(&max_smem, cudaDevAttrMaxSharedMemoryPerBlockOptin, dev));
  int cap = 2048;
  while (cap < 4 * h->K) cap <<= 1;
  B200_REQUIRE(cap <= 8192, "topK=%d too large for the top-K kernel (max 2048); use the dense path", h->K);
  h->cap = cap;
  h->cap_alloc = cap;
  const size_t staging = (size_t)STAGE_INTS * 4;
  {
    std::vector<int> hcnt((size_t)n_cols);
    B200_CUDA(cudaMemcpy(hcnt.data(), cnt_new.get(), sizeof(int) * (size_t)n_cols, cudaMemcpyDeviceToHost));
    int mx = 0;
    for (int j = 0; j < n_cols; ++j) mx = std::max(mx, hcnt[(size_t)j]);
    h->pack = h->binary && mx < 32768 && h->allow_pack;
  }
  auto windows_needed = [&](int cells_per_word, long long* cells_out) {
    int nw = 1;
    long long mc = 0;
    for (;; ++nw) {
      const size_t fixed = (size_t)cap * 8 + staging + (size_t)nw * (MAXTILES + 1) * 4 + sizeof(Shared) + 1024;
      mc = (((long long)max_smem - (long long)fixed) / 4) * cells_per_word;
      mc = std::min<long long>(mc, (long long)MAXTILES * THREADS * 4 * cells_per_word);
      B200_REQUIRE(mc >= 4096, "not enough shared memory (%d bytes) for the similarity kernel", max_smem);
      if ((long long)nw * mc >= n_cols) break;
    }
    *cells_out = mc;
    return nw;
  };
  long long max_cells = 0, max_cells_unpacked = 0;
  const int n_win_unpacked = windows_needed(1, &max_cells_unpacked);
  if (h->pack && windows_needed(2, &max_cells) >= n_win_unpacked) h->pack = false;
  const int cpw = h->pack ? 2 : 1;
  const int cpv = 4 * cpw;
  const int tile = THREADS * cpv;
  int n_win = windows_needed(cpw, &max_cells);
  int win = (n_cols + n_win - 1) / n_win;
  win = (win + cpv - 1) / cpv * cpv;
  if (win < cpv) win = cpv;
  h->n_win = n_win;
  h->win = win;
  h->acc_words = std::max(win / cpw, SBINS) + 4;
  h->smem_bytes = (size_t)h->acc_words * 4 + (size_t)cap * 8 + staging + (size_t)n_win * (MAXTILES + 1) * 4;
  B200_CUDA(cudaFuncSetAttribute(kernel_for(h->formula, h->binary, h->pack), cudaFuncAttributeMaxDynamicSharedMemorySize, (int)h->smem_bytes));
  h->tileB.alloc((size_t)n_win * (MAXTILES + 1));
  tile_bounds_kernel<<<div_up((long long)n_win * (MAXTILES + 1), 128), 128, 0, st>>>(h->BN.get(), n_cols, n_win, win, tile, h->tileB.get());
  count_launch();
  {
    const double avg_seg = nnz > 0 ? (double)nnz / (double)n_rows / (double)n_win : 1.0;
    const double chunks = avg_seg / (h->binary ? 4.0 : 2.0) + 1.0;
    int l2 = 1;
    while (l2 < 5 && (1 << l2) < chunks) ++l2;
    h->lpu_log2 = l2;
  }
  if (n_win > 1 || h->binary) {
    h->split.alloc((size_t)n_rows * (n_win + 1));
    const long long total = (long long)n_rows * (n_win + 1);
    split_kernel<<<div_up(total, 256), 256, 0, st>>>(h->csr_ptr.get(), h->csr_idx.get(), n_rows, n_win, win, h->split.get()); count_launch();
  }
  if (h->binary) {
    const long long n_seg = (long long)n_rows * n_win;
    B200_REQUIRE((long long)nnz + 3 * n_seg < (1ll << 31), "matrix too large for 32-bit positions in the padded row layout");
    DevBuf<int> len4((size_t)n_seg + 1), poff((size_t)n_seg + 1);
    B200_CUDA(cudaMemsetAsync(len4.get() + n_seg, 0, sizeof(int), st));
    seg_len_kernel<<<div_up(n_seg, 256), 256, 0, st>>>(h->split.get(), n_seg, n_win, len4.get()); count_launch();
    size_t tb = 0;
    B200_CUDA(cub::DeviceScan::ExclusiveSum(nullptr, tb, len4.get(), poff.get(), (int)(n_seg + 1), st));
    DevBuf<unsigned char> tmp(tb);
    B200_CUDA(cub::DeviceScan::ExclusiveSum(tmp.get(), tb, len4.get(), poff.get(), (int)(n_seg + 1), st)); count_launch();
    int total_pad = 0;
    B200_CUDA(cudaMemcpyAsync(&total_pad, poff.get() + n_seg, sizeof(int), cudaMemcpyDeviceToHost, st));
    B200_CUDA(cudaStreamSynchronize(st));
    DevBuf<int> idx_pad((size_t)total_pad + 8), split_pad((size_t)n_rows * (n_win + 1));
    seg_pad_kernel<<<div_up(n_seg * 8, 256), 256, 0, st>>>(h->split.get(), h->csr_idx.get(), poff.get(), n_seg, n_win, win, total_pad,
                                                          idx_pad.get(), split_pad.get()); count_launch();
    B200_CUDA(cudaStreamSynchronize(st));
    const bool f_ok_c = h->formula == F_PROD || h->formula == F_NONORM || h->formula == F_JACCARD || h->formula == F_DICE ||
                        (h->formula == F_TVERSKY && h->ta >= 0.f && h->tb >= 0.f);
    if (h->want_k1c && f_ok_c && nnz > 0 && n_cols >= h->k1c_min_cols) {
      const int win1 = ((n_cols + 7) / 8) * 8;
      DevBuf<int> sp1((size_t)n_rows * 2), len1((size_t)n_rows + 1), poff1((size_t)n_rows + 1), split1((size_t)n_rows * 2);
      split_kernel<<<div_up((long long)n_rows * 2, 256), 256, 0, st>>>(h->csr_ptr.get(), h->csr_idx.get(), n_rows, 1, win1, sp1.get()); count_launch();
      B200_CUDA(cudaMemsetAsync(len1.get() + n_rows, 0, sizeof(int), st));
      seg_len_kernel<<<div_up(n_rows, 256), 256, 0, st>>>(sp1.get(), n_rows, 1, len1.get()); count_launch();
      size_t tb1 = 0;
      B200_CUDA(cub::DeviceScan::ExclusiveSum(nullptr, tb1, len1.get(), poff1.get(), n_rows + 1, st));
      DevBuf<unsigned char> tmp1(tb1 + 16);
      B200_CUDA(cub::DeviceScan::ExclusiveSum(tmp1.get(), tb1, len1.get(), poff1.get(), n_rows + 1, st)); count_launch();
      int total1 = 0;
      B200_CUDA(cudaMemcpyAsync(&total1, poff1.get() + n_rows, sizeof(int), cudaMemcpyDeviceToHost, st));
      B200_CUDA(cudaStreamSynchronize(st));
      h->csr_idx1.alloc((size_t)total1 + 8);
      seg_pad_kernel<<<div_up((long long)n_rows * 8, 256), 256, 0, st>>>(sp1.get(), h->csr_idx.get(), poff1.get(), n_rows, 1, win1, total1,
                                                                        h->csr_idx1.get(), split1.get()); count_launch();
      h->csc_seg.alloc((size_t)nnz + 2);
      B200_CUDA(cudaMemsetAsync(h->csc_seg.get() + nnz, 0, 2 * sizeof(int2), st));
      k1d_csc_seg_kernel<<<GRID1D, 256, 0, st>>>(h->csc_idx.get(), split1.get(), h->csr_ptr.get(), nnz, h->csc_seg.get()); count_launch();
      B200_CUDA(cudaStreamSynchronize(st));
    }
    h->csr_idx = std::move(idx_pad);
    h->split = std::move(split_pad);
  }
  {
    DevBuf<unsigned long long> work((size_t)n_cols);
    col_work_kernel<<<div_up((long long)n_cols * 32, 256), 256, 0, st>>>(h->csc_ptr.get(), h->binary ? h->csc_idx.get() : nullptr,
                                                                        h->binary ? nullptr : h->csc_ent.get(), h->csr_ptr.get(), n_cols, work.get());
    count_launch();
    std::vector<unsigned long long> w_new((size_t)n_cols);
    std::vector<int> o2n((size_t)n_cols);
    B200_CUDA(cudaMemcpyAsync(w_new.data(), work.get(), sizeof(unsigned long long) * (size_t)n_cols, cudaMemcpyDeviceToHost, st));
    B200_CUDA(cudaMemcpyAsync(o2n.data(), h->old2new.get(), sizeof(int) * (size_t)n_cols, cudaMemcpyDeviceToHost, st));
    B200_CUDA(cudaStreamSynchronize(st));
    h->h_work.resize((size_t)n_cols);
    for (int c = 0; c < n_cols; ++c) h->h_work[(size_t)c] = w_new[(size_t)o2n[(size_t)c]];
  }
  if (!h->binary) h->csr_idx.release();
  h->counter.alloc(1);
  h->order.alloc((size_t)n_cols);
  h->k1c = false;
  if (h->csc_seg.n > 0) {
    const int win1 = ((n_cols + 7) / 8) * 8;
    h->ntile = (n_cols + (1 << D_TILE_LOG2) - 1) >> D_TILE_LOG2;
    h->bm_words = ((win1 / 8 + 1) + 3) / 4 * 4;
    const long long fixed = (long long)h->bm_words * 4 + ((long long)h->ntile + 1) * 4 + (long long)h->ntile * 4 + 32;
    cudaFuncAttributes fa{};
    B200_CUDA(cudaFuncGetAttributes(&fa, k1d_kernel_for(h->formula)));
    int dev = 0, sm_total = 0;
    B200_CUDA(cudaGetDevice(&dev));
    B200_CUDA(cudaDeviceGetAttribute(&sm_total, cudaDevAttrMaxSharedMemoryPerMultiprocessor, dev));
    const long long need_keys = (long long)h->K + (1ll << D_TILE_LOG2) + 128;
    for (int ctas = 2; ctas >= 1 && !h->k1c; --ctas) {
      long long avail = (long long)sm_total / ctas - (long long)fa.sharedSizeBytes - 1024;
      avail = std::min<long long>(avail, (long long)max_smem - (long long)fa.sharedSizeBytes);
      const long long keys = std::min<long long>((avail - fixed) / 8, 4 * D_THREADS);
      if (keys >= need_keys) {
        h->ctas_per_sm = ctas;
        h->cap_d = (int)keys;
        h->smem1_bytes = (size_t)(fixed + keys * 8);
        h->k1c = true;
      }
    }
    if (h->k1c) {
      h->tbnd.alloc((size_t)h->ntile + 1);
      k1d_tile_bounds_kernel<<<div_up(h->ntile + 1, 128), 128, 0, st>>>(h->BN.get(), n_cols, h->ntile, h->tbnd.get()); count_launch();
      h->fail.alloc(1);
      h->worklist.alloc((size_t)n_cols);
      h->h_old2new.resize((size_t)n_cols);
      h->h_csc_ptr.resize((size_t)n_cols + 1);
      B200_CUDA(cudaMemcpyAsync(h->h_old2new.data(), h->old2new.get(), sizeof(int) * (size_t)n_cols, cudaMemcpyDeviceToHost, st));
      B200_CUDA(cudaMemcpyAsync(h->h_csc_ptr.data(), h->csc_ptr.get(), sizeof(int) * ((size_t)n_cols + 1), cudaMemcpyDeviceToHost, st));
      B200_CUDA(cudaStreamSynchronize(st));
      B200_CUDA(cudaFuncSetAttribute(k1d_kernel_for(h->formula), cudaFuncAttributeMaxDynamicSharedMemorySize, (int)h->smem1_bytes));
      B200_CUDA(cudaFuncSetAttribute(k1d_kernel_for(h->formula), cudaFuncAttributePreferredSharedMemoryCarveout, (int)cudaSharedmemCarveoutMaxShared));
    }
  }
  if (!h->k1c) { h->csr_idx1.release(); h->csc_seg.release(); }
}

}

extern "C" {

int b200_sim_create(b200_sim_t* out, int64_t n_rows, int64_t n_cols, int64_t nnz, const int32_t* h_indptr,
                    const int32_t* h_indices, const float* h_data, int kind, int topK, float shrink, int normalize,
                    float asymmetric_alpha, float tversky_alpha, float tversky_beta, const float* h_row_weights,
                    void* stream) {
  if (out) *out = nullptr;
  b200_sim_s* h = nullptr;
  int rc = guarded([&] {
    B200_REQUIRE(out != nullptr, "b200_sim_create: out is NULL");
    B200_REQUIRE(n_rows > 0 && n_cols > 0 && nnz >= 0, "b200_sim_create: bad shape %lld x %lld nnz %lld",
                 (long long)n_rows, (long long)n_cols, (long long)nnz);
    B200_REQUIRE(n_rows < (1ll << 31) - 1 && n_cols < (1ll << 31) - 1 && nnz < (1ll << 31) - 1,
                 "b200_sim_create: int32 index range exceeded");
    B200_REQUIRE(kind >= B200_SIM_COSINE && kind <= B200_SIM_TVERSKY, "b200_sim_create: unknown similarity kind %d", kind);
    B200_REQUIRE(topK >= 1, "b200_sim_create: topK must be >= 1 (dense output goes through b200_sim_compute_dense)");
    B200_REQUIRE(h_indptr && (nnz == 0 || (h_indices && h_data)), "b200_sim_create: NULL input array");
    h = new b200_sim_s();
    h->allow_pack = getenv("B200REC_NO_PACK") == nullptr;
    if (const char* e = getenv("B200REC_K1C")) h->want_k1c = atoi(e) != 0;
    if (const char* e = getenv("B200REC_K1C_LAMBDA")) h->k1c_lambda = atof(e);
    if (const char* e = getenv("B200REC_K1C_MINCOLS")) h->k1c_min_cols = atoi(e);
    h->n_rows = (int)n_rows;
    h->n_cols = (int)n_cols;
    h->nnz = nnz;
    h->kind = kind;
    h->K = (int)std::min<int64_t>(topK, n_cols);
    const bool set_kind = kind == B200_SIM_JACCARD || kind == B200_SIM_DICE || kind == B200_SIM_TVERSKY;
    h->normalize = set_kind ? 0 : (normalize != 0);
    h->shrink = shrink;
    h->asym_alpha = asymmetric_alpha;
    h->ta = tversky_alpha;
    h->tb = tversky_beta;
    build(h, h_indptr, h_indices, h_data, h_row_weights, (cudaStream_t)stream);
    *out = h;
  });
  if (rc != B200_OK && h) delete h;
  return rc;
}

int b200_sim_create_scaled(b200_sim_t* out, int64_t n_rows, int64_t n_cols, int64_t nnz, const int32_t* h_indptr,
                           const int32_t* h_indices, const float* h_data, const float* h_A, const float* h_B, int topK,
                           void* stream) {
  if (out) *out = nullptr;
  b200_sim_s* h = nullptr;
  int rc = guarded([&] {
    B200_REQUIRE(out && h_indptr && h_A && h_B && (nnz == 0 || (h_indices && h_data)), "b200_sim_create_scaled: NULL argument");
    B200_REQUIRE(n_rows > 0 && n_cols > 0 && nnz >= 0 && nnz < (1ll << 31) - 1, "b200_sim_create_scaled: bad shape");
    B200_REQUIRE(topK >= 1, "b200_sim_create_scaled: topK must be >= 1");
    h = new b200_sim_s();
    h->n_rows = (int)n_rows; h->n_cols = (int)n_cols; h->nnz = nnz;
    h->kind = B200_SIM_COSINE;
    h->K = (int)std::min<int64_t>(topK, n_cols);
    h->scaled = true;
    h->h_A = h_A; h->h_B = h_B;
    build(h, h_indptr, h_indices, h_data, nullptr, (cudaStream_t)stream);
    h->h_A = h->h_B = nullptr;
    *out = h;
  });
  if (rc != B200_OK && h) delete h;
  return rc;
}

int b200_sim_create_euclidean(b200_sim_t* out, int64_t n_rows, int64_t n_cols, int64_t nnz, const int32_t* h_indptr,
                              const int32_t* h_indices, const float* h_data, int topK, float shrink, int normalize,
                              int normalize_avg_row, int distance_mode, void* stream) {
  if (out) *out = nullptr;
  b200_sim_s* h = nullptr;
  int rc = guarded([&] {
    B200_REQUIRE(out && h_indptr && (nnz == 0 || (h_indices && h_data)), "b200_sim_create_euclidean: NULL argument");
    B200_REQUIRE(n_rows > 0 && n_cols > 0 && nnz >= 0, "b200_sim_create_euclidean: bad shape %lld x %lld nnz %lld",
                 (long long)n_rows, (long long)n_cols, (long long)nnz);
    B200_REQUIRE(n_rows < (1ll << 31) - 1 && n_cols < (1ll << 31) - 1 && nnz < (1ll << 31) - 1,
                 "b200_sim_create_euclidean: int32 index range exceeded");
    B200_REQUIRE(topK >= 1, "b200_sim_create_euclidean: topK must be >= 1");
    B200_REQUIRE(distance_mode >= B200_EUCLID_EXP && distance_mode <= B200_EUCLID_LOG,
                 "b200_sim_create_euclidean: unknown similarity_from_distance_mode %d", distance_mode);
    h = new b200_sim_s();
    h->allow_pack = getenv("B200REC_NO_PACK") == nullptr;
    h->n_rows = (int)n_rows; h->n_cols = (int)n_cols; h->nnz = nnz;
    h->kind = B200_SIM_EUCLIDEAN;
    h->K = (int)std::min<int64_t>(topK, n_cols);
    h->normalize = 0;
    h->shrink = shrink;
    h->eu_mode = distance_mode; h->eu_norm = normalize != 0; h->eu_avg = normalize_avg_row != 0;
    build(h, h_indptr, h_indices, h_data, nullptr, (cudaStream_t)stream);
    *out = h;
  });
  if (rc != B200_OK && h) delete h;
  return rc;
}

int b200_sim_destroy(b200_sim_t h) {
  if (!h) return B200_OK;
  if (h->ev0) cudaEventDestroy(h->ev0);
  if (h->ev1) cudaEventDestroy(h->ev1);
  delete h;
  return B200_OK;
}

int b200_sim_info(b200_sim_t h, int* K, int* n_windows, int* window_cells, int* binary_path, int* signed_data) {
  return guarded([&] {
    B200_REQUIRE(h != nullptr, "b200_sim_info: NULL handle");
    if (K) *K = h->K;
    if (n_windows) *n_windows = h->n_win;
    if (window_cells) *window_cells = h->win;
    if (binary_path) *binary_path = h->binary ? (h->pack ? 2 : 1) : 0;
    if (signed_data) *signed_data = h->signed_data ? 1 : 0;
  });
}

struct PeerOut { int* idx; float* val; int* cnt; };

static void launch_topk(b200_sim_t h, int start_col, int end_col, int32_t* d_idx, float* d_val, int32_t* d_cnt, float* d_dense,
                        cudaStream_t st, const PeerOut* peers = nullptr, int n_peers = 0) {
  const int n_range = end_col - start_col;
  const bool use_k1c = h->k1c && d_dense == nullptr;
  if (h->order_lo != start_col || h->order_hi != end_col) {
    const unsigned long long* w = h->h_work.data() + start_col;
    std::vector<int> sparse;
    h->h_order.clear();
    for (int i = 0; i < n_range; ++i) {
      const bool sp = use_k1c && w[i] > 0 && (double)w[i] <= h->k1c_lambda * (double)h->n_cols;
      (sp ? sparse : h->h_order).push_back(i);
    }
    auto by_work = [w](int a, int b) { return w[a] > w[b]; };
    std::stable_sort(h->h_order.begin(), h->h_order.end(), by_work);
    std::stable_sort(sparse.begin(), sparse.end(), by_work);
    h->n_dense_last = (int)h->h_order.size();
    h->n_sparse_last = (int)sparse.size();
    if (!h->h_order.empty())
      B200_CUDA(cudaMemcpyAsync(h->order.get(), h->h_order.data(), sizeof(int) * h->h_order.size(), cudaMemcpyHostToDevice, st));
    std::vector<int4> wl(sparse.size());
    for (size_t k = 0; k < sparse.size(); ++k) {
      const int cn = h->h_old2new[(size_t)(start_col + sparse[k])];
      wl[k] = make_int4(cn, sparse[k], h->h_csc_ptr[(size_t)cn], h->h_csc_ptr[(size_t)cn + 1]);
    }
    if (!wl.empty()) B200_CUDA(cudaMemcpyAsync(h->worklist.get(), wl.data(), sizeof(int4) * wl.size(), cudaMemcpyHostToDevice, st));
    B200_CUDA(cudaStreamSynchronize(st));
    h->order_lo = start_col;
    h->order_hi = end_col;
  }
  const int n_sparse = use_k1c ? h->n_sparse_last : 0, n_dense = use_k1c ? h->n_dense_last : n_range;
  B200_CUDA(cudaMemsetAsync(h->counter.get(), 0, sizeof(int), st));
  KParams p;
  p.n_cols = h->n_cols; p.K = h->K; p.n_win = h->n_win; p.win = h->win; p.cap = h->cap; p.cap_alloc = h->cap_alloc;
  p.acc_cells = h->acc_words;
  p.lpu_log2 = h->lpu_log2;
  p.tileB = h->tileB.get();
  p.se = h->shrink + 1e-6f;
  p.shrink_div = h->shrink != 0.f ? h->shrink : 1.f;
  p.ta = h->ta; p.tb = h->tb;
  p.csr_ptr = h->csr_ptr.get(); p.csr_ent = h->csr_ent.get(); p.csr_idx = h->csr_idx.get();
  p.split = h->split.get();
  p.csc_ptr = h->csc_ptr.get(); p.csc_ent = h->csc_ent.get(); p.csc_idx = h->csc_idx.get();
  p.A = h->A.get(); p.BN = h->BN.get(); p.old2new = h->old2new.get();
  p.col_begin = start_col; p.n_range = n_dense;
  p.order = h->order.get();
  p.counter = h->counter.get();
  p.n_out = 1 + n_peers;
  p.o_idx[0] = d_idx; p.o_val[0] = d_val; p.o_cnt[0] = d_cnt;
  for (int r = 0; r < n_peers; ++r) { p.o_idx[1 + r] = peers[r].idx; p.o_val[1 + r] = peers[r].val; p.o_cnt[1 + r] = peers[r].cnt; }
  p.signed_data = (h->signed_data && h->formula != F_EUCLID) ? 1 : 0;
  p.eu_mode = h->eu_mode; p.eu_norm = h->eu_norm; p.eu_signed = h->signed_data ? 1 : 0;
  p.eu_div = h->eu_avg ? (float)h->n_rows : 1.f;
  p.eu_shrink = h->shrink;
  p.dense_out = d_dense;
  p.prof = h->prof_on ? h->prof.get() : nullptr;
  p.bm_words = h->bm_words; p.cap_d = h->cap_d; p.fail_every = h->fail_every; p.ntile = h->ntile; p.tbnd = h->tbnd.get();
  p.csr_idx1 = h->csr_idx1.get(); p.csc_seg = h->csc_seg.get(); p.worklist = h->worklist.get();
  p.redo = h->order.get(); p.fail = h->fail.get();
  p.n_range_dev = nullptr;
  B200_CUDA(cudaEventRecord(h->ev0, st));
  if (n_sparse > 0) {
    B200_CUDA(cudaMemcpyAsync(h->fail.get(), &h->n_dense_last, sizeof(int), cudaMemcpyHostToDevice, st));
    KParams q = p;
    q.n_range = n_sparse;
    k1d_kernel_for(h->formula)<<<std::min(n_sparse, h->n_sm * h->ctas_per_sm), D_THREADS, h->smem1_bytes, st>>>(q);
    B200_CUDA(cudaGetLastError());
    count_launch();
    B200_CUDA(cudaMemsetAsync(h->counter.get(), 0, sizeof(int), st));
    p.n_range_dev = h->fail.get();
  }
  if (n_dense > 0 || n_sparse > 0) {
    const int grid = n_sparse > 0 ? h->n_sm : std::min(n_dense, h->n_sm);
    kernel_for(h->formula, h->binary, h->pack)<<<grid, THREADS, h->smem_bytes, st>>>(p);
    B200_CUDA(cudaGetLastError());
    count_launch();
  }
  B200_CUDA(cudaEventRecord(h->ev1, st));
  h->timed = true;
}

int b200_sim_compute_device(b200_sim_t h, int start_col, int end_col, int32_t* d_idx, float* d_val, int32_t* d_cnt,
                            void* stream) {
  return guarded([&] {
    B200_REQUIRE(h != nullptr, "b200_sim_compute: NULL handle");
    B200_REQUIRE(0 <= start_col && start_col <= end_col && end_col <= h->n_cols, "b200_sim_compute: bad column range [%d,%d)",
                 start_col, end_col);
    if (end_col == start_col) return;
    B200_REQUIRE(d_idx && d_val && d_cnt, "b200_sim_compute: NULL output");
    launch_topk(h, start_col, end_col, d_idx, d_val, d_cnt, nullptr, (cudaStream_t)stream);
  });
}

int b200_sim_compute_peers_device(b200_sim_t h, int start_col, int end_col, int n_tables, void* const* d_tables, int64_t idx_offset,
                                  int64_t val_offset, int64_t cnt_offset, void* stream) {
  return guarded([&] {
    B200_REQUIRE(h != nullptr, "b200_sim_compute_peers: NULL handle");
    B200_REQUIRE(0 <= start_col && start_col <= end_col && end_col <= h->n_cols, "b200_sim_compute_peers: bad column range [%d,%d)",
                 start_col, end_col);
    B200_REQUIRE(n_tables >= 1 && n_tables <= B200_MAX_PEERS && d_tables != nullptr, "b200_sim_compute_peers: 1..%d tables", B200_MAX_PEERS);
    if (end_col == start_col) return;
    PeerOut out[B200_MAX_PEERS];
    for (int r = 0; r < n_tables; ++r) {
      B200_REQUIRE(d_tables[r] != nullptr, "b200_sim_compute_peers: NULL table");
      int32_t* base = reinterpret_cast<int32_t*>(d_tables[r]);
      out[r].idx = base + idx_offset + (int64_t)start_col * h->K;
      out[r].val = reinterpret_cast<float*>(base + val_offset) + (int64_t)start_col * h->K;
      out[r].cnt = base + cnt_offset + start_col;
    }
    launch_topk(h, start_col, end_col, out[0].idx, out[0].val, out[0].cnt, nullptr, (cudaStream_t)stream, out + 1, n_tables - 1);
  });
}

int b200_sim_compute_dense_device(b200_sim_t h, int start_col, int end_col, float* d_out, void* stream) {
  return guarded([&] {
    B200_REQUIRE(h != nullptr && d_out != nullptr, "b200_sim_compute_dense: NULL argument");
    B200_REQUIRE(h->formula != F_EUCLID, "b200_sim_compute_dense: the euclidean similarity has no dense output mode");
    B200_REQUIRE(0 <= start_col && start_col <= end_col && end_col <= h->n_cols, "b200_sim_compute_dense: bad column range [%d,%d)",
                 start_col, end_col);
    if (end_col == start_col) return;
    cudaStream_t st = (cudaStream_t)stream;
    B200_CUDA(cudaMemsetAsync(d_out, 0, sizeof(float) * (size_t)(end_col - start_col) * (size_t)h->n_cols, st));
    launch_topk(h, start_col, end_col, nullptr, nullptr, nullptr, d_out, st);
  });
}

int b200_sim_compute(b200_sim_t h, int start_col, int end_col, int32_t* h_idx, float* h_val, int32_t* h_cnt) {
  return guarded([&] {
    B200_REQUIRE(h != nullptr, "b200_sim_compute: NULL handle");
    B200_REQUIRE(0 <= start_col && start_col <= end_col && end_col <= h->n_cols, "b200_sim_compute: bad column range [%d,%d)",
                 start_col, end_col);
    const size_t n_range = (size_t)(end_col - start_col);
    if (n_range == 0) return;
    DevBuf<int> d_idx(n_range * h->K), d_cnt(n_range);
    DevBuf<float> d_val(n_range * h->K);
    int rc = b200_sim_compute_device(h, start_col, end_col, d_idx.get(), d_val.get(), d_cnt.get(), nullptr);
    if (rc != B200_OK) throw CudaFail{rc};
    B200_CUDA(cudaMemcpy(h_idx, d_idx.get(), sizeof(int) * n_range * h->K, cudaMemcpyDeviceToHost));
    B200_CUDA(cudaMemcpy(h_val, d_val.get(), sizeof(float) * n_range * h->K, cudaMemcpyDeviceToHost));
    B200_CUDA(cudaMemcpy(h_cnt, d_cnt.get(), sizeof(int) * n_range, cudaMemcpyDeviceToHost));
  });
}

int b200_sim_debug_set_cap(b200_sim_t h, int cap) {
  return guarded([&] {
    B200_REQUIRE(h != nullptr, "b200_sim_debug_set_cap: NULL handle");
    B200_REQUIRE(cap > h->K && cap <= h->cap_alloc, "b200_sim_debug_set_cap: cap must be in (K, %d]", h->cap_alloc);
    h->cap = cap;
  });
}

int b200_sim_debug_phase_cycles(b200_sim_t h, int enable, uint64_t* out8) {
  return guarded([&] {
    B200_REQUIRE(h != nullptr, "b200_sim_debug_phase_cycles: NULL handle");
    if (h->prof.n == 0) {
      h->prof.alloc(8);
      B200_CUDA(cudaMemset(h->prof.get(), 0, 8 * sizeof(unsigned long long)));
    }
    if (out8) {
      B200_CUDA(cudaDeviceSynchronize());
      B200_CUDA(cudaMemcpy(out8, h->prof.get(), 8 * sizeof(unsigned long long), cudaMemcpyDeviceToHost));
      B200_CUDA(cudaMemset(h->prof.get(), 0, 8 * sizeof(unsigned long long)));
    }
    h->prof_on = enable != 0;
  });
}

int b200_sim_debug_k1c(b200_sim_t h, int set_fail_every, int* enabled, int* ctas_per_sm, int* n_bitmap_cols, int* n_window_cols) {
  return guarded([&] {
    B200_REQUIRE(h != nullptr, "b200_sim_debug_k1c: NULL handle");
    if (set_fail_every >= 0 && h->k1c) h->fail_every = set_fail_every;
    if (enabled) *enabled = h->k1c ? 1 : 0;
    if (ctas_per_sm) *ctas_per_sm = h->k1c ? h->ctas_per_sm : 0;
    if (n_bitmap_cols) *n_bitmap_cols = h->n_sparse_last;
    if (n_window_cols) {
      *n_window_cols = h->n_dense_last;
      if (h->k1c && h->n_sparse_last > 0) {
        B200_CUDA(cudaDeviceSynchronize());
        B200_CUDA(cudaMemcpy(n_window_cols, h->fail.get(), sizeof(int), cudaMemcpyDeviceToHost));
      }
    }
  });
}

int b200_sim_last_kernel_ms(b200_sim_t h, float* ms) {
  return guarded([&] {
    B200_REQUIRE(h != nullptr && ms != nullptr, "b200_sim_last_kernel_ms: NULL argument");
    B200_REQUIRE(h->timed, "b200_sim_last_kernel_ms: no kernel launched yet");
    B200_CUDA(cudaEventSynchronize(h->ev1));
    B200_CUDA(cudaEventElapsedTime(ms, h->ev0, h->ev1));
  });
}

int b200_sim_col_work(b200_sim_t h, int64_t* out_n_cols) {
  return guarded([&] {
    B200_REQUIRE(h != nullptr && out_n_cols != nullptr, "b200_sim_col_work: NULL argument");
    for (int c = 0; c < h->n_cols; ++c) out_n_cols[c] = (int64_t)h->h_work[(size_t)c];
  });
}

int b200_sim_work(b200_sim_t h, int start_col, int end_col, int64_t* gathered_entries) {
  return guarded([&] {
    B200_REQUIRE(h != nullptr && gathered_entries != nullptr, "b200_sim_work: NULL argument");
    B200_REQUIRE(0 <= start_col && start_col <= end_col && end_col <= h->n_cols, "b200_sim_work: bad column range");
    unsigned long long s = 0;
    for (int c = start_col; c < end_col; ++c) s += h->h_work[(size_t)c];
    *gathered_entries = (int64_t)s;
  });
}

}
```

Before: 7.674 million.

## Warp-specialize sparse top-K kernel into gather and select warps with double-buffered bitmap

Splits the K1-D kernel into producer warps that gather co-occurrence counts into one of two shared bitmaps and consumer warps that run candidate scan and radix top-K select on the other, synchronized with named barriers. This overlaps the gather and select phases of consecutive items within one CTA per SM, instead of running two CTAs per SM that each do both phases in sequence. It also vectorizes the candidate sweep with warp prefix sums and unrolls the histogram loop. A single-buffer fallback kernel is kept for when shared memory cannot hold two bitmaps. The cost is doubled bitmap shared memory, fewer resident threads, and more complex barrier logic.

Result: slower. 7.157 million, median of 6 (-6.7%).

```diff
diff --git a/include/b200rec.h b/include/b200rec.h
--- a/include/b200rec.h
+++ b/include/b200rec.h
@@ -64,7 +64,7 @@
 
 int b200_sim_debug_phase_cycles(b200_sim_t h, int enable, uint64_t* out8);
 
-int b200_sim_debug_k1c(b200_sim_t h, int set_fail_every, int* enabled, int* ctas_per_sm, int* n_bitmap_cols, int* n_window_cols);
+int b200_sim_debug_k1c(b200_sim_t h, int set_fail_every, int* enabled, int* cols_per_sm, int* n_bitmap_cols, int* n_window_cols);
 
 int b200_sim_last_kernel_ms(b200_sim_t h, float* ms);
 int b200_sim_work(b200_sim_t h, int start_col, int end_col, int64_t* gathered_entries);
diff --git a/recsys2019_deeplearning_evaluation_b200/csrc/sim_k1d.cuh b/recsys2019_deeplearning_evaluation_b200/csrc/sim_k1d.cuh
--- a/recsys2019_deeplearning_evaluation_b200/csrc/sim_k1d.cuh
+++ b/recsys2019_deeplearning_evaluation_b200/csrc/sim_k1d.cuh
@@ -1,14 +1,47 @@
 
-constexpr int D_THREADS = 512;
-constexpr int D_WARPS = D_THREADS / 32;
-constexpr int D_ROWS = 4;
+#ifndef K1D_GATHER_WARPS
+#define K1D_GATHER_WARPS 20
+#endif
+#ifndef K1D_SELECT_WARPS
+#define K1D_SELECT_WARPS 12
+#endif
+#ifndef K1D_ROWS
+#define K1D_ROWS 4
+#endif
+constexpr int D_PWARPS = K1D_GATHER_WARPS;
+constexpr int D_CWARPS = K1D_SELECT_WARPS;
+constexpr int D_PTHREADS = D_PWARPS * 32;
+constexpr int D_CTHREADS = D_CWARPS * 32;
+constexpr int D_THREADS = D_PTHREADS + D_CTHREADS;
+constexpr int D_ROWS = K1D_ROWS;
+#ifndef K1D_SWEEP
+#define K1D_SWEEP 4
+#endif
+constexpr int D_SWEEP = K1D_SWEEP;
+constexpr int D_KEYQ = 8;
 constexpr int D_TILE_LOG2 = 10;
+static_assert(D_THREADS <= 1024 && D_CTHREADS >= 256 && D_PWARPS >= 1, "K1-D warp split");
+
+enum { BAR_FULL = 1, BAR_EMPTY = 3, BAR_GATHER = 5, BAR_SELECT = 6 };
+__device__ __forceinline__ void bar_sync(int id, int n) { asm volatile("bar.sync %0, %1;" ::"r"(id), "r"(n) : "memory"); }
+__device__ __forceinline__ void bar_arrive(int id, int n) { asm volatile("bar.arrive %0, %1;" ::"r"(id), "r"(n) : "memory"); }
+__device__ __forceinline__ void sel_sync() { bar_sync(BAR_SELECT, D_CTHREADS); }
+
+#define K1D_MARK(ph, lead)                                                   \
+  do {                                                                      \
+    if (p.prof && (lead)) {                                                 \
+      const long long _t = clock64();                                       \
+      atomicAdd(p.prof + (ph), (unsigned long long)(_t - prof_t));          \
+      prof_t = _t;                                                          \
+    }                                                                       \
+  } while (0)
 
 struct K1DShared {
-  int item, nbuf, cnt, adds, nibsum, tstop, chunk_end, chunk_cnt;
-  int need, digit, bincnt, ncand, expect;
+  int nbuf, cnt, nibsum, tstop, chunk_end, chunk_cnt;
+  int need, digit, bincnt, ncand;
   u64 kor, kand;
   int hist[256];
+  int item[2], adds[2];
 };
 
 __device__ __forceinline__ unsigned nib_ge3(unsigned w) { return (((w | (w >> 1)) >> 2) | (w & (w >> 1))) & 0x11111111u; }
@@ -22,19 +55,21 @@
   return (int)__dp4a(b, 0x01010101u, 0u);
 }
 
-__device__ u64 d_select(u64* buf, int n, int K, K1DShared* ds, int* n_out) {
-  const int tid = threadIdx.x;
-  __syncthreads();
+template <int NT, int BAR>
+__device__ u64 d_select(u64* buf, int n, int K, K1DShared* ds, int* n_out, const int tid) {
+  static_assert(NT >= 256, "one histogram bin per thread");
+  const auto sync = [] { bar_sync(BAR, NT); };
+  sync();
   if (n <= K) { *n_out = n; return 0ull; }
   {
     if (tid == 0) { ds->kor = 0ull; ds->kand = ~0ull; }
-    __syncthreads();
+    sync();
     u64 o = 0ull, a = ~0ull;
-    for (int q = tid; q < n; q += D_THREADS) { const u64 k = buf[q]; o |= k; a &= k; }
+    for (int q = tid; q < n; q += NT) { const u64 k = buf[q]; o |= k; a &= k; }
 #pragma unroll
     for (int off = 16; off > 0; off >>= 1) { o |= __shfl_xor_sync(0xffffffffu, o, off); a &= __shfl_xor_sync(0xffffffffu, a, off); }
     if ((tid & 31) == 0) { atomicOr(&ds->kor, o); atomicAnd(&ds->kand, a); }
-    __syncthreads();
+    sync();
   }
   const u64 diff = ds->kor ^ ds->kand;
   int pass = diff ? (63 - __clzll((long long)diff)) >> 3 : 0;
@@ -44,12 +79,17 @@
   for (; pass >= 0; --pass) {
     const int shift = pass * 8;
     if (tid < 256) ds->hist[tid] = 0;
-    __syncthreads();
-    for (int q = tid; q < n; q += D_THREADS) {
-      const u64 k = buf[q];
-      if (pass == 7 || (k >> (shift + 8)) == (prefix >> (shift + 8))) atomicAdd(&ds->hist[(int)((k >> shift) & 255ull)], one);
-    }
-    __syncthreads();
+    sync();
+    for (int q0 = tid; q0 < n; q0 += 4 * NT) {
+      u64 k[4];
+#pragma unroll
+      for (int u = 0; u < 4; ++u) k[u] = q0 + u * NT < n ? buf[q0 + u * NT] : 0ull;
+#pragma unroll
+      for (int u = 0; u < 4; ++u)
+        if (q0 + u * NT < n && (pass == 7 || (k[u] >> (shift + 8)) == (prefix >> (shift + 8))))
+          atomicAdd(&ds->hist[(int)((k[u] >> shift) & 255ull)], one);
+    }
+    sync();
     if (tid < 32) {
       int c[8], local = 0;
 #pragma unroll
@@ -67,125 +107,166 @@
         cum += c[b];
       }
     }
-    __syncthreads();
+    sync();
     prefix |= ((u64)ds->digit) << shift;
     need = ds->need;
     const int bincnt = ds->bincnt;
-    __syncthreads();
+    sync();
     if (bincnt == need) break;
   }
   const u64 thr = prefix;
-  u64 keep[8];
-#pragma unroll
-  for (int q = 0; q < 8; ++q) {
-    const int i = q * D_THREADS + tid;
+  u64 keep[D_KEYQ];
+#pragma unroll
+  for (int q = 0; q < D_KEYQ; ++q) {
+    const int i = q * NT + tid;
     const u64 k = i < n ? buf[i] : 0ull;
     keep[q] = k >= thr ? k : 0ull;
   }
   if (tid == 0) ds->cnt = 0;
-  __syncthreads();
-#pragma unroll
-  for (int q = 0; q < 8; ++q)
+  sync();
+#pragma unroll
+  for (int q = 0; q < D_KEYQ; ++q)
     if (keep[q]) buf[atomicAdd(&ds->cnt, 1)] = keep[q];
-  __syncthreads();
+  sync();
   *n_out = ds->cnt;
   return thr;
 }
 
 template <int F>
-__global__ void __launch_bounds__(D_THREADS, 2) sim_k1d_kernel(const KParams p) {
+__global__ void __launch_bounds__(D_THREADS, 1) sim_k1d_kernel(const KParams p) {
   extern __shared__ __align__(16) unsigned char smem_raw[];
   __shared__ K1DShared ds;
-  const int tid = threadIdx.x, lane = tid & 31, warp = tid >> 5;
+  const int lane = threadIdx.x & 31, warp = threadIdx.x >> 5;
   const int W = p.bm_words;
   const int Wr = (p.n_cols + 7) >> 3;
   const int ntile = p.ntile;
-  unsigned* acc = reinterpret_cast<unsigned*>(smem_raw);
-  u64* buf = reinterpret_cast<u64*>(smem_raw + (size_t)W * 4);
+  unsigned* acc0 = reinterpret_cast<unsigned*>(smem_raw);
+  u64* buf = reinterpret_cast<u64*>(smem_raw + (size_t)2 * W * 4);
   float* tbs = reinterpret_cast<float*>(buf + p.cap_d);
   int* tcnt = reinterpret_cast<int*>(tbs + ntile + 1);
 
-  for (int i = tid; i < W; i += D_THREADS) acc[i] = 0u;
-  for (int i = tid; i <= ntile; i += D_THREADS) tbs[i] = p.tbnd[i];
-  for (int i = tid; i < ntile; i += D_THREADS) tcnt[i] = 0;
+  for (int i = threadIdx.x; i < 2 * W; i += D_THREADS) acc0[i] = 0u;
+  for (int i = threadIdx.x; i <= ntile; i += D_THREADS) tbs[i] = p.tbnd[i];
+  for (int i = threadIdx.x; i < ntile; i += D_THREADS) tcnt[i] = 0;
+  __syncthreads();
   long long prof_t = p.prof ? clock64() : 0;
   const int K = p.K;
 
-  for (;;) {
-    __syncthreads();
-    if (tid == 0) { ds.item = atomicAdd(p.counter, 1); ds.nbuf = 0; ds.adds = 0; ds.nibsum = 0; ds.ncand = 0; }
-    __syncthreads();
-    const int item = ds.item;
+  if (warp < D_PWARPS) {
+    const int tid = threadIdx.x;
+    int next_item = tid == 0 ? atomicAdd(p.counter, 1) : 0;
+    for (int b = 0;; b ^= 1) {
+      bar_sync(BAR_EMPTY + b, D_THREADS);
+      K1D_MARK(0, tid == 0);
+      if (tid == 0) { ds.item[b] = next_item; ds.adds[b] = 0; }
+      bar_sync(BAR_GATHER, D_PTHREADS);
+      const int item = ds.item[b];
+      if (item >= p.n_range) { bar_arrive(BAR_FULL + b, D_THREADS); break; }
+      if (tid == 0) next_item = atomicAdd(p.counter, 1);
+      const int4 wi = __ldg(p.worklist + item);
+      const int col = wi.x, cs = wi.z, ce = wi.w;
+      unsigned* acc = acc0 + (size_t)b * W;
+      int expect = 0;
+      for (int k0 = cs + warp * 32; k0 < ce; k0 += D_PWARPS * 32) {
+        const int nrows = min(32, ce - k0);
+        int2 seg = make_int2(0, 0);
+        if (lane < nrows) {
+          seg = __ldg(p.csc_seg + k0 + lane);
+          expect += 4 * (seg.y >> 2) - (seg.y & 3) - 1;
+        }
+        for (int r0 = 0; r0 < nrows; r0 += D_ROWS) {
+          int4 v[D_ROWS];
+          int rs[D_ROWS], rn[D_ROWS];
+#pragma unroll
+          for (int q = 0; q < D_ROWS; ++q) {
+            const int r = r0 + q;
+            rs[q] = __shfl_sync(0xffffffffu, seg.x, r & 31);
+            rn[q] = r < nrows ? (__shfl_sync(0xffffffffu, seg.y, r & 31) >> 2) : 0;
+            if (lane < rn[q]) v[q] = __ldg(reinterpret_cast<const int4*>(p.csr_idx1) + (size_t)rs[q] + lane);
+          }
+#pragma unroll
+          for (int q = 0; q < D_ROWS; ++q) {
+            int c0 = 0;
+            for (;;) {
+              if (c0 + lane < rn[q]) {
+                const int jj[4] = {v[q].x, v[q].y, v[q].z, v[q].w};
+#pragma unroll
+                for (int c = 0; c < 4; ++c) {
+                  const int j = jj[c];
+                  if ((unsigned)j < (unsigned)p.n_cols && j != col) atomicAdd(&acc[j >> 3], 1u << ((j & 7) << 2));
+                }
+              }
+              c0 += 32;
+              if (c0 >= rn[q]) break;
+              if (c0 + lane < rn[q]) v[q] = __ldg(reinterpret_cast<const int4*>(p.csr_idx1) + (size_t)rs[q] + c0 + lane);
+            }
+          }
+        }
+      }
+      expect = __reduce_add_sync(0xffffffffu, expect);
+      if (lane == 0 && expect) atomicAdd(&ds.adds[b], expect);
+      bar_arrive(BAR_FULL + b, D_THREADS);
+      K1D_MARK(1, tid == 0);
+    }
+    return;
+  }
+
+  const int tid = threadIdx.x - D_PTHREADS;
+  bar_arrive(BAR_EMPTY + 0, D_THREADS);
+  bar_arrive(BAR_EMPTY + 1, D_THREADS);
+  for (int b = 0;; b ^= 1) {
+    bar_sync(BAR_FULL + b, D_THREADS);
+    K1D_MARK(2, tid == 0);
+    const int item = ds.item[b];
     if (item >= p.n_range) break;
     const int4 wi = __ldg(p.worklist + item);
-    const int col = wi.x, lc = wi.y, cs = wi.z, ce = wi.w;
+    const int col = wi.x, lc = wi.y;
     const size_t out_base = (size_t)lc * K;
     const float Ai = p.A[col];
-
-    int expect = 0;
-    for (int k0 = cs + warp * 32; k0 < ce; k0 += D_WARPS * 32) {
-      const int nrows = min(32, ce - k0);
-      int2 seg = make_int2(0, 0);
-      if (lane < nrows) {
-        seg = __ldg(p.csc_seg + k0 + lane);
-        expect += 4 * (seg.y >> 2) - (seg.y & 3) - 1;
-      }
-      for (int r0 = 0; r0 < nrows; r0 += D_ROWS) {
-        int4 v[D_ROWS];
-        int rs[D_ROWS], rn[D_ROWS];
-#pragma unroll
-        for (int q = 0; q < D_ROWS; ++q) {
-          const int r = r0 + q;
-          rs[q] = __shfl_sync(0xffffffffu, seg.x, r & 31);
-          rn[q] = r < nrows ? (__shfl_sync(0xffffffffu, seg.y, r & 31) >> 2) : 0;
-          if (lane < rn[q]) v[q] = __ldg(reinterpret_cast<const int4*>(p.csr_idx1) + (size_t)rs[q] + lane);
-        }
-#pragma unroll
-        for (int q = 0; q < D_ROWS; ++q) {
-          int c0 = 0;
-          for (;;) {
-            if (c0 + lane < rn[q]) {
-              const int jj[4] = {v[q].x, v[q].y, v[q].z, v[q].w};
-#pragma unroll
-              for (int c = 0; c < 4; ++c) {
-                const int j = jj[c];
-                if ((unsigned)j < (unsigned)p.n_cols && j != col) atomicAdd(&acc[j >> 3], 1u << ((j & 7) << 2));
-              }
-            }
-            c0 += 32;
-            if (c0 >= rn[q]) break;
-            if (c0 + lane < rn[q]) v[q] = __ldg(reinterpret_cast<const int4*>(p.csr_idx1) + (size_t)rs[q] + c0 + lane);
-          }
-        }
-      }
-    }
-    expect = __reduce_add_sync(0xffffffffu, expect);
-    if (lane == 0 && expect) atomicAdd(&ds.adds, expect);
-    __syncthreads();
-    PROF_MARK(1);
+    unsigned* acc = acc0 + (size_t)b * W;
+    if (tid == 0) { ds.nbuf = 0; ds.nibsum = 0; ds.ncand = 0; }
+    sel_sync();
 
     {
       int ns = 0;
       unsigned* cand = reinterpret_cast<unsigned*>(buf);
-      const int cand_cap = p.cap_d;
+      const int n4 = (Wr + 3) >> 2;
       const uint4* acc4 = reinterpret_cast<const uint4*>(acc);
-      for (int i4 = tid; i4 < ((Wr + 3) >> 2); i4 += D_THREADS) {
-        const uint4 w4 = acc4[i4];
-        if (!(w4.x | w4.y | w4.z | w4.w)) continue;
-        const unsigned ww[4] = {w4.x, w4.y, w4.z, w4.w};
-        unsigned bytes = 0u, any = 0u, m[4];
-#pragma unroll
-        for (int e = 0; e < 4; ++e) {
-          bytes += (ww[e] & 0x0F0F0F0Fu) + ((ww[e] >> 4) & 0x0F0F0F0Fu);
-          m[e] = nib_ge3(ww[e]);
-          any |= m[e];
-        }
-        ns += (int)__dp4a(bytes, 0x01010101u, 0u);
-        if (any) {
-          const int c3 = __popc(m[0]) + __popc(m[1]) + __popc(m[2]) + __popc(m[3]);
-          atomicAdd(&tcnt[(i4 * 4) >> (D_TILE_LOG2 - 3)], c3);
-          int pos = atomicAdd(&ds.ncand, c3);
-          if (pos + c3 <= cand_cap) {
+      for (int v0 = tid - lane; v0 < n4; v0 += D_SWEEP * D_CTHREADS) {
+        uint4 w4[D_SWEEP];
+#pragma unroll
+        for (int u = 0; u < D_SWEEP; ++u) {
+          const int i4 = v0 + u * D_CTHREADS + lane;
+          w4[u] = i4 < n4 ? acc4[i4] : make_uint4(0u, 0u, 0u, 0u);
+        }
+#pragma unroll
+        for (int u = 0; u < D_SWEEP; ++u) {
+          const int i4 = v0 + u * D_CTHREADS + lane;
+          const unsigned ww[4] = {w4[u].x, w4[u].y, w4[u].z, w4[u].w};
+          unsigned bytes = 0u, m[4];
+          int c3 = 0;
+#pragma unroll
+          for (int e = 0; e < 4; ++e) {
+            bytes += (ww[e] & 0x0F0F0F0Fu) + ((ww[e] >> 4) & 0x0F0F0F0Fu);
+            m[e] = nib_ge3(ww[e]);
+            c3 += __popc(m[e]);
+          }
+          ns += (int)__dp4a(bytes, 0x01010101u, 0u);
+          int incl = c3;
+#pragma unroll
+          for (int off = 1; off < 32; off <<= 1) {
+            const int t = __shfl_up_sync(0xffffffffu, incl, off);
+            if (lane >= off) incl += t;
+          }
+          const int tot = __shfl_sync(0xffffffffu, incl, 31);
+          if (tot == 0) continue;
+          int base = 0;
+          if (lane == 31) {
+            atomicAdd(&tcnt[(v0 + u * D_CTHREADS) >> (D_TILE_LOG2 - 5)], tot);
+            base = atomicAdd(&ds.ncand, tot);
+          }
+          int pos = __shfl_sync(0xffffffffu, base, 31) + incl - c3;
+          if (c3 && pos + c3 <= p.cap_d) {
 #pragma unroll
             for (int e = 0; e < 4; ++e) {
               unsigned mm = m[e];
@@ -201,16 +282,18 @@
       ns = __reduce_add_sync(0xffffffffu, ns);
       if (lane == 0 && ns) atomicAdd(&ds.nibsum, ns);
     }
-    __syncthreads();
+    sel_sync();
+    K1D_MARK(3, tid == 0);
     const bool forced = p.fail_every > 0 && (lc % p.fail_every) == 0;
-    if (ds.nibsum != ds.adds || forced) {
-      __syncthreads();
+    if (ds.nibsum != ds.adds[b] || forced) {
+      sel_sync();
       if (tid == 0) p.redo[atomicAdd(p.fail, 1)] = lc;
-      for (int i = tid; i < (W >> 2); i += D_THREADS) reinterpret_cast<int4*>(acc)[i] = make_int4(0, 0, 0, 0);
-      for (int i = tid; i < ntile; i += D_THREADS) tcnt[i] = 0;
+      for (int i = tid; i < (W >> 2); i += D_CTHREADS) reinterpret_cast<int4*>(acc)[i] = make_int4(0, 0, 0, 0);
+      for (int i = tid; i < ntile; i += D_CTHREADS) tcnt[i] = 0;
+      bar_arrive(BAR_EMPTY + b, D_THREADS);
+      K1D_MARK(3, tid == 0);
       continue;
     }
-    PROF_MARK(2);
 
     u64 thr = 0ull;
     int n_have = 0;
@@ -218,10 +301,10 @@
     const bool collected = n3 <= p.cap_d;
     if (collected) {
       const unsigned* cand = reinterpret_cast<const unsigned*>(buf);
-      u64 keys[4];
-#pragma unroll
-      for (int q = 0; q < 4; ++q) {
-        const int t = q * D_THREADS + tid;
+      u64 keys[D_KEYQ];
+#pragma unroll
+      for (int q = 0; q < D_KEYQ; ++q) {
+        const int t = q * D_CTHREADS + tid;
         keys[q] = 0ull;
         if (t < n3) {
           const unsigned cd = cand[t];
@@ -230,18 +313,18 @@
           if (sv > 0.f) keys[q] = (((u64)__float_as_uint(sv)) << 32) | (u64)(0xFFFFFFFFu - (unsigned)bn.y);
         }
       }
-      __syncthreads();
-#pragma unroll
-      for (int q = 0; q < 4; ++q)
+      sel_sync();
+#pragma unroll
+      for (int q = 0; q < D_KEYQ; ++q)
         if (keys[q]) buf[atomicAdd(&ds.nbuf, 1)] = keys[q];
-      for (int i = tid; i < ntile; i += D_THREADS) tcnt[i] = 0;
-      __syncthreads();
+      for (int i = tid; i < ntile; i += D_CTHREADS) tcnt[i] = 0;
+      sel_sync();
       n_have = ds.nbuf;
       if (n_have >= K) {
         const float fl = sim_value<F>(p, 3.f, Ai, tbs[ntile]) * (1.f - 1e-6f);
         if (fl > 0.f) thr = ((u64)__float_as_uint(fl)) << 32;
       }
-      PROF_MARK(3);
+      K1D_MARK(4, tid == 0);
     }
 #pragma unroll 1
     for (int level = collected ? 2 : 3; level >= 1; --level) {
@@ -252,22 +335,22 @@
         } else {
           const float tsim = __uint_as_float((unsigned)(thr >> 32));
           if (tid == 0) ds.tstop = ntile;
-          __syncthreads();
-          for (int t = tid; t < ntile; t += D_THREADS)
+          sel_sync();
+          for (int t = tid; t < ntile; t += D_CTHREADS)
             if (!(sim_value<F>(p, (float)level, Ai, tbs[t]) >= tsim)) atomicMin(&ds.tstop, t);
-          __syncthreads();
+          sel_sync();
           t_end = ds.tstop;
-          __syncthreads();
+          sel_sync();
         }
         if (t_end == 0) continue;
         const int w_end = min(Wr, t_end << (D_TILE_LOG2 - 3));
-        for (int i = tid; i < w_end; i += D_THREADS) {
+        for (int i = tid; i < w_end; i += D_CTHREADS) {
           const unsigned w = acc[i];
           if (!w) continue;
           const int c = __popc(nib_level(w, level));
           if (c) atomicAdd(&tcnt[i >> (D_TILE_LOG2 - 3)], c);
         }
-        __syncthreads();
+        sel_sync();
       }
       int t0 = 0;
       while (t0 < t_end) {
@@ -277,20 +360,20 @@
           ds.chunk_end = t1;
           ds.chunk_cnt = c;
         }
-        __syncthreads();
+        sel_sync();
         const int t1 = ds.chunk_end;
         if (t1 == t0) {
           int kept;
-          const u64 t2 = d_select(buf, n_have, K, &ds, &kept);
+          const u64 t2 = d_select<D_CTHREADS, BAR_SELECT>(buf, n_have, K, &ds, &kept, tid);
           thr = max(thr, t2);
           if (tid == 0) ds.nbuf = kept;
           n_have = kept;
-          __syncthreads();
+          sel_sync();
           continue;
         }
         if (ds.chunk_cnt > 0) {
           const int w_lo = t0 << (D_TILE_LOG2 - 3), w_hi = min(Wr, t1 << (D_TILE_LOG2 - 3));
-          for (int i = w_lo + tid; i < w_hi; i += D_THREADS) {
+          for (int i = w_lo + tid; i < w_hi; i += D_CTHREADS) {
             const unsigned w = acc[i];
             if (!w) continue;
             unsigned m = nib_level(w, level);
@@ -306,11 +389,270 @@
             }
           }
         }
+        sel_sync();
+        n_have = ds.nbuf;
+        t0 = t1;
+      }
+      for (int i = tid; i < ntile; i += D_CTHREADS) tcnt[i] = 0;
+      sel_sync();
+      if (n_have >= K) {
+        if (level == 3 && thr == 0ull) {
+          const float fl = sim_value<F>(p, 3.f, Ai, tbs[ntile]) * (1.f - 1e-6f);
+          if (fl > 0.f) thr = ((u64)__float_as_uint(fl)) << 32;
+        } else if (level == 2 && n_have > K) {
+          int kept;
+          const u64 t2 = d_select<D_CTHREADS, BAR_SELECT>(buf, n_have, K, &ds, &kept, tid);
+          thr = max(thr, t2);
+          if (tid == 0) ds.nbuf = kept;
+          n_have = kept;
+          sel_sync();
+        }
+      }
+      K1D_MARK(level == 3 ? 4 : 5, tid == 0);
+    }
+
+    {
+      int kept;
+      d_select<D_CTHREADS, BAR_SELECT>(buf, n_have, K, &ds, &kept, tid);
+      n_have = kept;
+    }
+    for (int t = tid; t < n_have; t += D_CTHREADS) {
+      const u64 k64 = buf[t];
+      emit_entry(p, out_base + t, (int)(0xFFFFFFFFu - (unsigned)k64), __uint_as_float((unsigned)(k64 >> 32)));
+    }
+    for (int t = n_have + tid; t < K; t += D_CTHREADS) {
+      emit_entry(p, out_base + t, -1, 0.f);
+    }
+    if (tid == 0) emit_count(p, lc, n_have);
+    for (int i = tid; i < (W >> 2); i += D_CTHREADS) reinterpret_cast<int4*>(acc)[i] = make_int4(0, 0, 0, 0);
+    bar_arrive(BAR_EMPTY + b, D_THREADS);
+    K1D_MARK(6, tid == 0);
+  }
+}
+
+constexpr int D1_THREADS = 512;
+constexpr int D1_WARPS = D1_THREADS / 32;
+constexpr int D1_ROWS = 4;
+
+template <int F>
+__global__ void __launch_bounds__(D1_THREADS, 2) sim_k1d_single_kernel(const KParams p) {
+  extern __shared__ __align__(16) unsigned char smem_raw[];
+  __shared__ K1DShared ds;
+  const int tid = threadIdx.x, lane = tid & 31, warp = tid >> 5;
+  const int W = p.bm_words;
+  const int Wr = (p.n_cols + 7) >> 3;
+  const int ntile = p.ntile;
+  unsigned* acc = reinterpret_cast<unsigned*>(smem_raw);
+  u64* buf = reinterpret_cast<u64*>(smem_raw + (size_t)W * 4);
+  float* tbs = reinterpret_cast<float*>(buf + p.cap_d);
+  int* tcnt = reinterpret_cast<int*>(tbs + ntile + 1);
+
+  for (int i = tid; i < W; i += D1_THREADS) acc[i] = 0u;
+  for (int i = tid; i <= ntile; i += D1_THREADS) tbs[i] = p.tbnd[i];
+  for (int i = tid; i < ntile; i += D1_THREADS) tcnt[i] = 0;
+  long long prof_t = p.prof ? clock64() : 0;
+  const int K = p.K;
+
+  for (;;) {
+    __syncthreads();
+    if (tid == 0) { ds.item[0] = atomicAdd(p.counter, 1); ds.nbuf = 0; ds.adds[0] = 0; ds.nibsum = 0; ds.ncand = 0; }
+    __syncthreads();
+    const int item = ds.item[0];
+    if (item >= p.n_range) break;
+    const int4 wi = __ldg(p.worklist + item);
+    const int col = wi.x, lc = wi.y, cs = wi.z, ce = wi.w;
+    const size_t out_base = (size_t)lc * K;
+    const float Ai = p.A[col];
+
+    int expect = 0;
+    for (int k0 = cs + warp * 32; k0 < ce; k0 += D1_WARPS * 32) {
+      const int nrows = min(32, ce - k0);
+      int2 seg = make_int2(0, 0);
+      if (lane < nrows) {
+        seg = __ldg(p.csc_seg + k0 + lane);
+        expect += 4 * (seg.y >> 2) - (seg.y & 3) - 1;
+      }
+      for (int r0 = 0; r0 < nrows; r0 += D1_ROWS) {
+        int4 v[D1_ROWS];
+        int rs[D1_ROWS], rn[D1_ROWS];
+#pragma unroll
+        for (int q = 0; q < D1_ROWS; ++q) {
+          const int r = r0 + q;
+          rs[q] = __shfl_sync(0xffffffffu, seg.x, r & 31);
+          rn[q] = r < nrows ? (__shfl_sync(0xffffffffu, seg.y, r & 31) >> 2) : 0;
+          if (lane < rn[q]) v[q] = __ldg(reinterpret_cast<const int4*>(p.csr_idx1) + (size_t)rs[q] + lane);
+        }
+#pragma unroll
+        for (int q = 0; q < D1_ROWS; ++q) {
+          int c0 = 0;
+          for (;;) {
+            if (c0 + lane < rn[q]) {
+              const int jj[4] = {v[q].x, v[q].y, v[q].z, v[q].w};
+#pragma unroll
+              for (int c = 0; c < 4; ++c) {
+                const int j = jj[c];
+                if ((unsigned)j < (unsigned)p.n_cols && j != col) atomicAdd(&acc[j >> 3], 1u << ((j & 7) << 2));
+              }
+            }
+            c0 += 32;
+            if (c0 >= rn[q]) break;
+            if (c0 + lane < rn[q]) v[q] = __ldg(reinterpret_cast<const int4*>(p.csr_idx1) + (size_t)rs[q] + c0 + lane);
+          }
+        }
+      }
+    }
+    expect = __reduce_add_sync(0xffffffffu, expect);
+    if (lane == 0 && expect) atomicAdd(&ds.adds[0], expect);
+    __syncthreads();
+    PROF_MARK(1);
+
+    {
+      int ns = 0;
+      unsigned* cand = reinterpret_cast<unsigned*>(buf);
+      const int cand_cap = p.cap_d;
+      const uint4* acc4 = reinterpret_cast<const uint4*>(acc);
+      for (int i4 = tid; i4 < ((Wr + 3) >> 2); i4 += D1_THREADS) {
+        const uint4 w4 = acc4[i4];
+        if (!(w4.x | w4.y | w4.z | w4.w)) continue;
+        const unsigned ww[4] = {w4.x, w4.y, w4.z, w4.w};
+        unsigned bytes = 0u, any = 0u, m[4];
+#pragma unroll
+        for (int e = 0; e < 4; ++e) {
+          bytes += (ww[e] & 0x0F0F0F0Fu) + ((ww[e] >> 4) & 0x0F0F0F0Fu);
+          m[e] = nib_ge3(ww[e]);
+          any |= m[e];
+        }
+        ns += (int)__dp4a(bytes, 0x01010101u, 0u);
+        if (any) {
+          const int c3 = __popc(m[0]) + __popc(m[1]) + __popc(m[2]) + __popc(m[3]);
+          atomicAdd(&tcnt[(i4 * 4) >> (D_TILE_LOG2 - 3)], c3);
+          int pos = atomicAdd(&ds.ncand, c3);
+          if (pos + c3 <= cand_cap) {
+#pragma unroll
+            for (int e = 0; e < 4; ++e) {
+              unsigned mm = m[e];
+              while (mm) {
+                const int q = (__ffs(mm) - 1) >> 2;
+                mm &= mm - 1;
+                cand[pos++] = ((unsigned)((i4 * 4 + e) * 8 + q) << 4) | ((ww[e] >> (q << 2)) & 15u);
+              }
+            }
+          }
+        }
+      }
+      ns = __reduce_add_sync(0xffffffffu, ns);
+      if (lane == 0 && ns) atomicAdd(&ds.nibsum, ns);
+    }
+    __syncthreads();
+    const bool forced = p.fail_every > 0 && (lc % p.fail_every) == 0;
+    if (ds.nibsum != ds.adds[0] || forced) {
+      __syncthreads();
+      if (tid == 0) p.redo[atomicAdd(p.fail, 1)] = lc;
+      for (int i = tid; i < (W >> 2); i += D1_THREADS) reinterpret_cast<int4*>(acc)[i] = make_int4(0, 0, 0, 0);
+      for (int i = tid; i < ntile; i += D1_THREADS) tcnt[i] = 0;
+      continue;
+    }
+    PROF_MARK(2);
+
+    u64 thr = 0ull;
+    int n_have = 0;
+    const int n3 = ds.ncand;
+    const bool collected = n3 <= p.cap_d;
+    if (collected) {
+      const unsigned* cand = reinterpret_cast<const unsigned*>(buf);
+      u64 keys[4];
+#pragma unroll
+      for (int q = 0; q < 4; ++q) {
+        const int t = q * D1_THREADS + tid;
+        keys[q] = 0ull;
+        if (t < n3) {
+          const unsigned cd = cand[t];
+          const int2 bn = __ldg(p.BN + (cd >> 4));
+          const float sv = sim_value<F>(p, (float)(cd & 15u), Ai, __int_as_float(bn.x));
+          if (sv > 0.f) keys[q] = (((u64)__float_as_uint(sv)) << 32) | (u64)(0xFFFFFFFFu - (unsigned)bn.y);
+        }
+      }
+      __syncthreads();
+#pragma unroll
+      for (int q = 0; q < 4; ++q)
+        if (keys[q]) buf[atomicAdd(&ds.nbuf, 1)] = keys[q];
+      for (int i = tid; i < ntile; i += D1_THREADS) tcnt[i] = 0;
+      __syncthreads();
+      n_have = ds.nbuf;
+      if (n_have >= K) {
+        const float fl = sim_value<F>(p, 3.f, Ai, tbs[ntile]) * (1.f - 1e-6f);
+        if (fl > 0.f) thr = ((u64)__float_as_uint(fl)) << 32;
+      }
+      PROF_MARK(3);
+    }
+#pragma unroll 1
+    for (int level = collected ? 2 : 3; level >= 1; --level) {
+      int t_end = ntile;
+      if (level < 3) {
+        if (thr == 0ull) {
+          t_end = ntile;
+        } else {
+          const float tsim = __uint_as_float((unsigned)(thr >> 32));
+          if (tid == 0) ds.tstop = ntile;
+          __syncthreads();
+          for (int t = tid; t < ntile; t += D1_THREADS)
+            if (!(sim_value<F>(p, (float)level, Ai, tbs[t]) >= tsim)) atomicMin(&ds.tstop, t);
+          __syncthreads();
+          t_end = ds.tstop;
+          __syncthreads();
+        }
+        if (t_end == 0) continue;
+        const int w_end = min(Wr, t_end << (D_TILE_LOG2 - 3));
+        for (int i = tid; i < w_end; i += D1_THREADS) {
+          const unsigned w = acc[i];
+          if (!w) continue;
+          const int c = __popc(nib_level(w, level));
+          if (c) atomicAdd(&tcnt[i >> (D_TILE_LOG2 - 3)], c);
+        }
+        __syncthreads();
+      }
+      int t0 = 0;
+      while (t0 < t_end) {
+        if (tid == 0) {
+          int t1 = t0, c = 0;
+          while (t1 < t_end && n_have + c + tcnt[t1] <= p.cap_d) { c += tcnt[t1]; ++t1; }
+          ds.chunk_end = t1;
+          ds.chunk_cnt = c;
+        }
+        __syncthreads();
+        const int t1 = ds.chunk_end;
+        if (t1 == t0) {
+          int kept;
+          const u64 t2 = d_select<D1_THREADS, 0>(buf, n_have, K, &ds, &kept, tid);
+          thr = max(thr, t2);
+          if (tid == 0) ds.nbuf = kept;
+          n_have = kept;
+          __syncthreads();
+          continue;
+        }
+        if (ds.chunk_cnt > 0) {
+          const int w_lo = t0 << (D_TILE_LOG2 - 3), w_hi = min(Wr, t1 << (D_TILE_LOG2 - 3));
+          for (int i = w_lo + tid; i < w_hi; i += D1_THREADS) {
+            const unsigned w = acc[i];
+            if (!w) continue;
+            unsigned m = nib_level(w, level);
+            while (m) {
+              const int q = (__ffs(m) - 1) >> 2;
+              m &= m - 1;
+              const int j = i * 8 + q;
+              const float d = (float)((w >> (q << 2)) & 15u);
+              const int2 bn = __ldg(p.BN + j);
+              const float sv = sim_value<F>(p, d, Ai, __int_as_float(bn.x));
+              const u64 key = (((u64)__float_as_uint(sv)) << 32) | (u64)(0xFFFFFFFFu - (unsigned)bn.y);
+              if (sv > 0.f && key >= thr) buf[atomicAdd(&ds.nbuf, 1)] = key;
+            }
+          }
+        }
         __syncthreads();
         n_have = ds.nbuf;
         t0 = t1;
       }
-      for (int i = tid; i < ntile; i += D_THREADS) tcnt[i] = 0;
+      for (int i = tid; i < ntile; i += D1_THREADS) tcnt[i] = 0;
       __syncthreads();
       if (n_have >= K) {
         if (level == 3 && thr == 0ull) {
@@ -318,7 +660,7 @@
           if (fl > 0.f) thr = ((u64)__float_as_uint(fl)) << 32;
         } else if (level == 2 && n_have > K) {
           int kept;
-          const u64 t2 = d_select(buf, n_have, K, &ds, &kept);
+          const u64 t2 = d_select<D1_THREADS, 0>(buf, n_have, K, &ds, &kept, tid);
           thr = max(thr, t2);
           if (tid == 0) ds.nbuf = kept;
           n_have = kept;
@@ -330,21 +672,22 @@
 
     {
       int kept;
-      d_select(buf, n_have, K, &ds, &kept);
+      d_select<D1_THREADS, 0>(buf, n_have, K, &ds, &kept, tid);
       n_have = kept;
     }
-    for (int t = tid; t < n_have; t += D_THREADS) {
+    for (int t = tid; t < n_have; t += D1_THREADS) {
       const u64 k64 = buf[t];
       emit_entry(p, out_base + t, (int)(0xFFFFFFFFu - (unsigned)k64), __uint_as_float((unsigned)(k64 >> 32)));
     }
-    for (int t = n_have + tid; t < K; t += D_THREADS) {
+    for (int t = n_have + tid; t < K; t += D1_THREADS) {
       emit_entry(p, out_base + t, -1, 0.f);
     }
     if (tid == 0) emit_count(p, lc, n_have);
-    for (int i = tid; i < (W >> 2); i += D_THREADS) reinterpret_cast<int4*>(acc)[i] = make_int4(0, 0, 0, 0);
+    for (int i = tid; i < (W >> 2); i += D1_THREADS) reinterpret_cast<int4*>(acc)[i] = make_int4(0, 0, 0, 0);
     PROF_MARK(6);
   }
 }
+
 
 __global__ void k1d_tile_bounds_kernel(const int2* __restrict__ BN, int n_cols, int ntile, float* tb) {
   const int t = blockIdx.x * blockDim.x + threadIdx.x;
diff --git a/recsys2019_deeplearning_evaluation_b200/csrc/sim_topk.cu b/recsys2019_deeplearning_evaluation_b200/csrc/sim_topk.cu
--- a/recsys2019_deeplearning_evaluation_b200/csrc/sim_topk.cu
+++ b/recsys2019_deeplearning_evaluation_b200/csrc/sim_topk.cu
@@ -1095,7 +1095,7 @@
   DevBuf<int2> csc_seg;
   DevBuf<float> tbnd;
   DevBuf<int4> worklist;
-  int bm_words = 0, cap_d = 0, fail_every = 0, ctas_per_sm = 0, ntile = 0;
+  int bm_words = 0, cap_d = 0, fail_every = 0, nbuf = 0, ntile = 0;
   size_t smem1_bytes = 0;
   double k1c_lambda = 0.75;
   int k1c_min_cols = 32768;
@@ -1134,13 +1134,13 @@
   }
 }
 
-sim_kernel_t k1d_kernel_for(int formula) {
+sim_kernel_t k1d_kernel_for(int formula, int nbuf) {
   switch (formula) {
-    case F_PROD: return sim_k1d_kernel<F_PROD>;
-    case F_NONORM: return sim_k1d_kernel<F_NONORM>;
-    case F_JACCARD: return sim_k1d_kernel<F_JACCARD>;
-    case F_DICE: return sim_k1d_kernel<F_DICE>;
-    default: return sim_k1d_kernel<F_TVERSKY>;
+    case F_PROD: return nbuf == 2 ? sim_k1d_kernel<F_PROD> : sim_k1d_single_kernel<F_PROD>;
+    case F_NONORM: return nbuf == 2 ? sim_k1d_kernel<F_NONORM> : sim_k1d_single_kernel<F_NONORM>;
+    case F_JACCARD: return nbuf == 2 ? sim_k1d_kernel<F_JACCARD> : sim_k1d_single_kernel<F_JACCARD>;
+    case F_DICE: return nbuf == 2 ? sim_k1d_kernel<F_DICE> : sim_k1d_single_kernel<F_DICE>;
+    default: return nbuf == 2 ? sim_k1d_kernel<F_TVERSKY> : sim_k1d_single_kernel<F_TVERSKY>;
   }
 }
 
@@ -1410,19 +1410,15 @@
     const int win1 = ((n_cols + 7) / 8) * 8;
     h->ntile = (n_cols + (1 << D_TILE_LOG2) - 1) >> D_TILE_LOG2;
     h->bm_words = ((win1 / 8 + 1) + 3) / 4 * 4;
-    const long long fixed = (long long)h->bm_words * 4 + ((long long)h->ntile + 1) * 4 + (long long)h->ntile * 4 + 32;
-    cudaFuncAttributes fa{};
-    B200_CUDA(cudaFuncGetAttributes(&fa, k1d_kernel_for(h->formula)));
-    int dev = 0, sm_total = 0;
-    B200_CUDA(cudaGetDevice(&dev));
-    B200_CUDA(cudaDeviceGetAttribute(&sm_total, cudaDevAttrMaxSharedMemoryPerMultiprocessor, dev));
     const long long need_keys = (long long)h->K + (1ll << D_TILE_LOG2) + 128;
-    for (int ctas = 2; ctas >= 1 && !h->k1c; --ctas) {
-      long long avail = (long long)sm_total / ctas - (long long)fa.sharedSizeBytes - 1024;
-      avail = std::min<long long>(avail, (long long)max_smem - (long long)fa.sharedSizeBytes);
-      const long long keys = std::min<long long>((avail - fixed) / 8, 4 * D_THREADS);
+    for (int nbuf = 2; nbuf >= 1 && !h->k1c; --nbuf) {
+      cudaFuncAttributes fa{};
+      B200_CUDA(cudaFuncGetAttributes(&fa, k1d_kernel_for(h->formula, nbuf)));
+      const long long fixed = (long long)nbuf * h->bm_words * 4 + ((long long)h->ntile + 1) * 4 + (long long)h->ntile * 4 + 32;
+      const long long avail = (long long)max_smem - (long long)fa.sharedSizeBytes;
+      const long long keys = std::min<long long>((avail - fixed) / 8, nbuf == 2 ? (long long)D_KEYQ * D_CTHREADS : 4ll * D1_THREADS);
       if (keys >= need_keys) {
-        h->ctas_per_sm = ctas;
+        h->nbuf = nbuf;
         h->cap_d = (int)keys;
         h->smem1_bytes = (size_t)(fixed + keys * 8);
         h->k1c = true;
@@ -1438,8 +1434,7 @@
       B200_CUDA(cudaMemcpyAsync(h->h_old2new.data(), h->old2new.get(), sizeof(int) * (size_t)n_cols, cudaMemcpyDeviceToHost, st));
       B200_CUDA(cudaMemcpyAsync(h->h_csc_ptr.data(), h->csc_ptr.get(), sizeof(int) * ((size_t)n_cols + 1), cudaMemcpyDeviceToHost, st));
       B200_CUDA(cudaStreamSynchronize(st));
-      B200_CUDA(cudaFuncSetAttribute(k1d_kernel_for(h->formula), cudaFuncAttributeMaxDynamicSharedMemorySize, (int)h->smem1_bytes));
-      B200_CUDA(cudaFuncSetAttribute(k1d_kernel_for(h->formula), cudaFuncAttributePreferredSharedMemoryCarveout, (int)cudaSharedmemCarveoutMaxShared));
+      B200_CUDA(cudaFuncSetAttribute(k1d_kernel_for(h->formula, h->nbuf), cudaFuncAttributeMaxDynamicSharedMemorySize, (int)h->smem1_bytes));
     }
   }
   if (!h->k1c) { h->csr_idx1.release(); h->csc_seg.release(); }
@@ -1624,7 +1619,7 @@
     B200_CUDA(cudaMemcpyAsync(h->fail.get(), &h->n_dense_last, sizeof(int), cudaMemcpyHostToDevice, st));
     KParams q = p;
     q.n_range = n_sparse;
-    k1d_kernel_for(h->formula)<<<std::min(n_sparse, h->n_sm * h->ctas_per_sm), D_THREADS, h->smem1_bytes, st>>>(q);
+    k1d_kernel_for(h->formula, h->nbuf)<<<std::min(n_sparse, h->n_sm), h->nbuf == 2 ? D_THREADS : D1_THREADS, h->smem1_bytes, st>>>(q);
     B200_CUDA(cudaGetLastError());
     count_launch();
     B200_CUDA(cudaMemsetAsync(h->counter.get(), 0, sizeof(int), st));
@@ -1726,12 +1721,12 @@
   });
 }
 
-int b200_sim_debug_k1c(b200_sim_t h, int set_fail_every, int* enabled, int* ctas_per_sm, int* n_bitmap_cols, int* n_window_cols) {
+int b200_sim_debug_k1c(b200_sim_t h, int set_fail_every, int* enabled, int* cols_per_sm, int* n_bitmap_cols, int* n_window_cols) {
   return guarded([&] {
     B200_REQUIRE(h != nullptr, "b200_sim_debug_k1c: NULL handle");
     if (set_fail_every >= 0 && h->k1c) h->fail_every = set_fail_every;
     if (enabled) *enabled = h->k1c ? 1 : 0;
-    if (ctas_per_sm) *ctas_per_sm = h->k1c ? h->ctas_per_sm : 0;
+    if (cols_per_sm) *cols_per_sm = h->k1c ? h->nbuf : 0;
     if (n_bitmap_cols) *n_bitmap_cols = h->n_sparse_last;
     if (n_window_cols) {
       *n_window_cols = h->n_dense_last;
```
